# Clemapfel/kmer_index

Hardware: AMD Instinct MI355X
Metric: M queries/sec, DNA4 k=10 exact-match batch search, 1e8-bp text (higher is better)
Workload: dtype u32/u64

## Files before the change

### include/kmx.h

```cpp
#ifndef KMX_H
#define KMX_H

#include <stddef.h>
#include <stdint.h>

#ifdef __cplusplus
extern "C" {
#endif

#define KMX_VERSION 5
#define KMX_MAX_KS 32
#define KMX_MAX_DEVICES 16
#define KMX_QUERY_SIZE_RANGE 10000
#define KMX_SUBK_FANOUT_LIMIT 10000000ull

typedef enum kmx_status {
    KMX_OK = 0,
    KMX_ERR_INVALID_ARGUMENT = 1,
    KMX_ERR_HIP = 2,
    KMX_ERR_OUT_OF_MEMORY = 3,
    KMX_ERR_NO_DEVICE = 4,
    KMX_ERR_TOO_LARGE = 5
} kmx_status;

// ... 34 lines not shown
} kmx_options;

#define KMX_SEARCH_DEFAULT 0u
#define KMX_SEARCH_KEEP_MASKS 1u
#define KMX_SEARCH_COUNT_ONLY 2u
#define KMX_SEARCH_ASYNC 4u
#define KMX_SEARCH_REFERENCE_PLAN 8u

typedef struct kmx_index kmx_index;
typedef struct kmx_result kmx_result;

#define KMX_N_KERNELS 16
typedef struct kmx_kernel_stat {
    const char* name;
    uint64_t launches;
    double total_ms;
} kmx_kernel_stat;

kmx_status kmx_index_build(const uint8_t* ranks, uint64_t n, uint32_t sigma, const uint32_t* ks,
                           uint32_t n_ks, const kmx_options* opts, kmx_index** out);
void kmx_index_free(kmx_index* index);

kmx_status kmx_index_save(const kmx_index* index, const char* path);
kmx_status kmx_index_load(const char* path, const kmx_options* opts, kmx_index** out);

kmx_status kmx_index_info(const kmx_index* index, uint64_t* n, uint32_t* sigma, uint32_t* n_ks,
                          uint32_t* ks , uint32_t* table_kinds ,
                          uint64_t* device_bytes);

kmx_status kmx_index_memory(const kmx_index* index, uint64_t* positions, uint64_t* aligned_copy, uint64_t* cells,
                            uint64_t* prefix_levels, uint64_t* tables);

kmx_status kmx_index_extend_query_size_range(kmx_index* index, uint32_t new_maximum);

kmx_status kmx_plan(const uint32_t* ks, uint32_t n_ks, uint32_t range, uint8_t* use_multi,
                    uint32_t* nk_off, uint32_t* nk_flat, uint64_t cap, uint64_t* n_flat);

kmx_status kmx_plan_engine(const uint32_t* ks, uint32_t n_ks, uint32_t range, uint32_t sigma, uint32_t* k_used);

kmx_status kmx_choose_best_k(const uint64_t* query_lengths, uint64_t n_lengths, uint32_t n_k, uint32_t* ks_out);

uint64_t kmx_fast_pow(uint64_t base, uint8_t exp);

kmx_status kmx_search_batch(const kmx_index* index, const uint8_t* qranks, const uint64_t* qoff,
                            uint64_t nq, uint32_t flags, kmx_result** out);

kmx_status kmx_search_batch_device(const kmx_index* index, const void* d_qranks, const void* d_qoff,
                                   uint64_t nq, uint32_t flags, void* stream, kmx_result** inout);

kmx_status kmx_result_counts(const kmx_result* r, uint64_t* nq, uint64_t* n_hits, uint64_t* n_exact,
                             uint64_t* n_stitch, uint64_t* n_prefix, uint64_t* n_error);
kmx_status kmx_result_view_device(const kmx_result* r, const uint64_t** d_hit_off,
                                  const uint32_t** d_positions, const uint8_t** d_status);
kmx_status kmx_result_view(kmx_result* r, const uint64_t** hit_off, const uint32_t** positions,
                           const uint8_t** status, const uint8_t** kinds);

kmx_status kmx_result_parts(const kmx_result* r, uint32_t* n_parts);
kmx_status kmx_result_part_view_device(const kmx_result* r, uint32_t part, int32_t* device, uint64_t* q_begin, uint64_t* q_end,
                                       const uint64_t** d_hit_off, const uint32_t** d_positions, const uint8_t** d_status);
kmx_status kmx_index_devices(const kmx_index* index, uint32_t* n_devices, int32_t* devices);

kmx_status kmx_result_gather_device(kmx_result* r, int32_t dst_device, const uint64_t** d_hit_off, const uint32_t** d_positions,
                                    const uint8_t** d_status);

kmx_status kmx_result_masks(kmx_result* r, const uint64_t** mask_base, const uint64_t** mask_words,
                            const uint32_t** cand_count, const uint64_t** cand_src);
kmx_status kmx_index_arena_host(const kmx_index* index, const uint32_t** arena, uint64_t* n_elems);

kmx_status kmx_index_bucket_host(const kmx_index* index, uint32_t k, const uint8_t* ranks, const uint32_t** positions,
                                 uint32_t* count);

kmx_status kmx_index_levels(const kmx_index* index, uint32_t* levels);

#define KMX_PATH_INFO 1
typedef struct kmx_index_path_info {
    uint32_t struct_size;
    uint32_t fill_slots;
    uint32_t fill_nontemporal;
    uint32_t rec64;
    uint32_t tiny_cells;
    uint32_t scan_tile;
    uint32_t n_ks;
    uint32_t cell_shift[KMX_MAX_KS];
} kmx_index_path_info;
kmx_status kmx_index_paths(const kmx_index* index, kmx_index_path_info* out);

typedef struct kmx_result_path_info {
    uint32_t struct_size;
    uint32_t small;
    uint32_t lookup_items;
    uint32_t lookup_pairs;
    uint32_t deferred_long;
    uint32_t tile_q_source;
    uint32_t spec_fill;
    uint32_t spec_ok;
    uint32_t fill_blocks;
    uint32_t fill_tiles;
    uint32_t prefix_plain;
    uint32_t prefix_small;
    uint32_t prefix_merge_small;
    uint32_t prefix_mid;
    uint32_t prefix_long;
    uint32_t prefix_large_chunks;
    uint64_t prefix_large_elems;
} kmx_result_path_info;
#define KMX_TILE_Q_NONE 0u
#define KMX_TILE_Q_PARTITION 1u
#define KMX_TILE_Q_SCAN 2u
kmx_status kmx_result_paths(const kmx_result* r, kmx_result_path_info* out);

void kmx_result_free(kmx_result* r);

#define KMX_APPROX_MAX_SUBST 3
#define KMX_APPROX_EDIT 1u
typedef struct kmx_approx_result kmx_approx_result;
kmx_status kmx_search_approx(const kmx_index* index, const uint8_t* qranks, const uint64_t* qoff, uint64_t nq,
                             uint32_t max_subst, uint32_t flags, kmx_approx_result** out);
kmx_status kmx_approx_counts(const kmx_approx_result* r, uint64_t* nq, uint64_t* n_hits, uint64_t* n_candidates,
                             uint32_t* n_chunks);
kmx_status kmx_approx_view(kmx_approx_result* r, const uint64_t** hit_off, const uint32_t** positions,
                           const uint8_t** mismatches, const uint8_t** status);
kmx_status kmx_approx_lengths(kmx_approx_result* r, const uint32_t** lengths);
void kmx_approx_free(kmx_approx_result* r);

#define KMX_APPROX_BOTH_STRANDS 1
kmx_status kmx_search_approx_strands(const kmx_index* index, const uint8_t* qranks, const uint64_t* qoff, uint64_t nq,
                                     uint32_t max_subst, uint32_t flags, const uint8_t* complement,
                                     kmx_approx_result** out);
kmx_status kmx_approx_strands(kmx_approx_result* r, const uint8_t** strands);

#define KMX_APPROX_REPORT 1
#define KMX_APPROX_LOCI 2u
#define KMX_APPROX_BEST 4u
typedef struct kmx_approx_options {
    uint32_t struct_size;
    uint32_t max_subst;
    uint32_t flags;
    uint32_t max_hits;
    const uint8_t* complement;
} kmx_approx_options;
kmx_status kmx_search_approx_opts(const kmx_index* index, const uint8_t* qranks, const uint64_t* qoff, uint64_t nq,
                                  const kmx_approx_options* options, kmx_approx_result** out);
kmx_status kmx_approx_found(kmx_approx_result* r, const uint64_t** found );

kmx_status kmx_index_text(const kmx_index* index, uint8_t* out_ranks, uint64_t n, uint64_t* packed_bytes);

kmx_status kmx_stats_enable(kmx_index* index, int enable);
kmx_status kmx_stats_get(kmx_index* index, kmx_kernel_stat* stats , uint32_t* n);
kmx_status kmx_stats_reset(kmx_index* index);

kmx_status kmx_debug_words(const kmx_index* index, uint64_t* words16);

const char* kmx_last_error(void);
const char* kmx_status_string(kmx_status s);
uint32_t kmx_version(void);

#ifdef __cplusplus
}
#endif
#endif
```

### kmer_index_amd/csrc/kmx_capi.hip

```cpp
#include <hip/hip_runtime.h>

#include <algorithm>
#include <atomic>
#include <cstddef>
#include <cstdio>
#include <cstdlib>
#include <cstring>
#include <memory>
#include <mutex>
#include <string>
#include <system_error>
#include <thread>
#include <vector>

#include "kmx_approx.h"
#include "kmx_host.h"
#include "kmx_kernels.h"

namespace {

thread_local std::string g_err;

kmx_status fail(kmx_status st, const std::string& msg)
{
// ... 74 lines not shown
        }
        p = nullptr; cap = 0; pinned = false;
    }
    template <typename T> T* as() const { return static_cast<T*>(p); }
};

enum KernelId {
    K_LOOKUP = 0, K_SCAN, K_PARTITION, K_FILL, K_VALIDATE, K_COMPACT, K_PREFIX_LEN, K_MERGE_PASS,
    K_PREFIX_SORT_SMALL, K_PREFIX_MERGE_SMALL, K_PREFIX_SORT_BLOCK, K_SMALL, K_PREFIX_BANDS, K_PREFIX_SPLIT, K_COUNT
};
const char* const kKernelNames[K_COUNT] = {
    "k_lookup", "k_scan", "k_partition", "k_fill", "k_validate", "k_compact",
    "k_prefix_len", "k_prefix_merge_pass", "k_prefix_sort_small", "k_prefix_merge_small", "k_prefix_sort_block", "k_small", "k_prefix_bands", "k_prefix_split"};

struct Stats {
    bool enabled = false;
    std::mutex mu;
    struct Pending { int id; hipEvent_t a, b; };
    std::vector<Pending> pending;
    std::vector<hipEvent_t> pool;
    uint64_t launches[K_COUNT] = {};
    double ms[K_COUNT] = {};

    hipEvent_t get()
    {
        if (!pool.empty()) { hipEvent_t e = pool.back(); pool.pop_back(); return e; }
        hipEvent_t e = nullptr;
        (void)hipEventCreate(&e);
        return e;
    }
    void drain()
    {
        for (auto& p : pending) {
            (void)hipEventSynchronize(p.b);
            float t = 0.f;
            if (hipEventElapsedTime(&t, p.a, p.b) == hipSuccess) { ms[p.id] += t; launches[p.id] += 1; }
            pool.push_back(p.a);
            pool.push_back(p.b);
        }
        pending.clear();
    }
    void destroy()
    {
        drain();
        for (auto e : pool) (void)hipEventDestroy(e);
        pool.clear();
    }
};

}

struct ResultPool {
    std::mutex mu;
    std::vector<kmx_result*> idle;
    std::vector<kmx_result*> pending;
    bool closed = false;
};
constexpr size_t kPoolMaxResults = 8;
constexpr size_t kPoolMaxBytes = size_t(256) << 20;
constexpr size_t kSmallView = size_t(256) << 10;

struct kmx_index {
    std::shared_ptr<ResultPool> pool = std::make_shared<ResultPool>();
    int device = 0;
    uint64_t n = 0;
    uint32_t sigma = 0;
    uint32_t range = KMX_QUERY_SIZE_RANGE;
    std::vector<uint32_t> ks;
    std::vector<uint32_t> table_kinds;
    std::vector<void*> allocs;
    uint64_t device_bytes = 0;
    uint64_t bytes_positions = 0, bytes_aligned = 0, bytes_cells = 0, bytes_levels = 0;
    KmxIndexDev* d_index = nullptr;
    KmxIndexDev* d_index_fast = nullptr;
    const KmxPlanEntry* d_plan_fast = nullptr;
    const uint32_t* d_arena = nullptr;
    unsigned long long* d_dbg = nullptr;
    struct ElemSizes { size_t n_offs, n_slots, n_ukeys, n_aoffs; };
    std::vector<ElemSizes> elem_sizes;
    std::vector<uint8_t> tail;
    KmxIndexDev h_header{};
    kmx::FillVariant fill_variant{12, true};
    bool rec32 = true;
    bool tiny_cells = false;
    bool broken = false;
    std::vector<uint32_t> host_arena;
    Stats stats;
    struct HostDir {
        std::once_flag once;
        kmx_status st = KMX_OK;
        std::string err;
        std::vector<uint32_t> offs;
        std::vector<uint64_t> ukeys;
    };
    std::unique_ptr<HostDir[]> host_dirs;
    std::vector<kmx_index*> peers;
    std::unique_ptr<kmx::PackedText> text = std::make_unique<kmx::PackedText>();
    size_t n_replicas() const { return 1 + peers.size(); }
    kmx_index* replica(size_t i) { return i ? peers[i - 1] : this; }
};

struct SearchCtx {
    kmx_index* ix = nullptr;
    const uint8_t* qr = nullptr;
    const uint64_t* qo = nullptr;
    hipStream_t s = nullptr;
    uint64_t tile_cap = 0, spec_tiles = 0;
    bool spec_fill = false;
    bool pending = false;
};

struct kmx_result {
    const kmx_index* index = nullptr;
    int device = 0;
    hipStream_t stream = nullptr;
    uint32_t flags = 0;
    uint64_t nq = 0, n_hits = 0, n_exact = 0, n_stitch = 0, n_prefix = 0, n_error = 0, n_none = 0;
    uint64_t n_mask_words = 0;
    DevBuf src, cnt, c0, aux, key, p1, kind, status, stitch_list, prefix_list, short_list, hit_off, bsum, ctr, tile_q, out,
        mask_words, stitch_hits, plen, poff, ptmp, pitems, pbands, pcuts, pbanded, psplits, ptiles, pscnt, pscratch, pmid, in_qranks, in_qoff;
    unsigned long long* h_ctr = nullptr;
    HostBuf h_hit_off, h_positions, h_status, h_kinds, h_mask_base, h_mask_words, h_cand_count, h_cand_src, h_small;
    uint64_t* v_hit_off = nullptr; uint32_t* v_positions = nullptr; uint8_t* v_status = nullptr; uint8_t* v_kinds = nullptr;
    const uint64_t* m_base = nullptr; const uint64_t* m_words = nullptr; const uint32_t* m_ccnt = nullptr; const uint64_t* m_csrc = nullptr;
    uint32_t ctr_phase = 0;
    bool ctr_clean = false;
    HostBuf mailbox, small_in;
    DevBuf small_xchg;
    bool small_valid = false;
    bool host_valid = false, host_masks_valid = false;
    bool last_had_stitch = false;
    bool last_had_long = false;
    bool last_had_pairs = false;
    struct PathRec { uint32_t small = 0, items = 0, pairs = 0, defer_long = 0, tile_q_source = 0, spec_fill = 0, spec_ok = 0, fill_blocks = 0, fill_tiles = 0;
                     uint32_t p_plain = 0, p_small = 0, p_merge = 0, p_mid = 0, p_long = 0, p_chunks = 0; uint64_t p_elems = 0; };
    PathRec path;
    std::shared_ptr<ResultPool> pool;
    SearchCtx ctx;
    hipEvent_t done = nullptr;
    bool quiesced = true;
    hipStream_t own_stream = nullptr;
    std::vector<kmx_result*> parts;
    std::vector<uint64_t> part_q0;
    std::vector<uint64_t> part_w0;
    bool chunked = false;
    bool host_chunk = false;
    kmx_result* worker = nullptr;
    kmx_result* worker2 = nullptr;
    DevBuf g_hit_off, g_out, g_status;
    int gather_device = -1;
    hipStream_t gather_stream = nullptr;

    size_t device_bytes() const
    {
        size_t b = 0;
        for (const DevBuf* d : {&src, &cnt, &c0, &aux, &key, &p1, &kind, &status, &stitch_list, &prefix_list, &short_list, &hit_off, &bsum, &ctr,
                                &tile_q, &out, &mask_words, &stitch_hits, &plen, &poff, &ptmp, &pitems, &pbands, &pcuts, &pbanded, &psplits, &ptiles, &pscnt, &pscratch, &pmid, &in_qranks, &in_qoff, &small_xchg})
            b += d->cap;
        return b;
    }

    void release()
    {
        for (DevBuf* b : {&src, &cnt, &c0, &aux, &key, &p1, &kind, &status, &stitch_list, &prefix_list, &short_list, &hit_off, &bsum, &ctr,
                          &tile_q, &out, &mask_words, &stitch_hits, &plen, &poff, &ptmp, &pitems, &pbands, &pcuts, &pbanded, &psplits, &ptiles, &pscnt, &pscratch, &pmid, &in_qranks, &in_qoff, &small_xchg})
            b->release();
        for (HostBuf* b : {&h_hit_off, &h_positions, &h_status, &h_kinds, &h_mask_base, &h_mask_words, &h_cand_count, &h_cand_src, &h_small, &mailbox, &small_in})
            b->release();
        if (h_ctr) (void)hipHostFree(h_ctr);
        h_ctr = nullptr;
        if (done) (void)hipEventDestroy(done);
        done = nullptr;
        if (own_stream) (void)hipStreamDestroy(own_stream);
        own_stream = nullptr;
        if (gather_device >= 0) {
            int cur = 0;
            const bool have = hipGetDevice(&cur) == hipSuccess;
            (void)hipSetDevice(gather_device);
            g_hit_off.release(); g_out.release(); g_status.release();
            if (gather_stream) (void)hipStreamDestroy(gather_stream);
            gather_stream = nullptr;
            gather_device = -1;
            if (have) (void)hipSetDevice(cur);
        }
    }
};

namespace {

kmx_result* take_result(kmx_index* ix)
{
    kmx_result* r = nullptr;
    {
        std::lock_guard<std::mutex> lock(ix->pool->mu);
        if (!ix->pool->idle.empty()) { r = ix->pool->idle.back(); ix->pool->idle.pop_back(); }
    }
    if (!r) r = new kmx_result();
    r->pool = ix->pool;
    return r;
}

template <typename F>
void timed(kmx_index* ix, int id, hipStream_t s, F&& launch)
{
    if (!ix->stats.enabled) { launch(); return; }
    std::lock_guard<std::mutex> lock(ix->stats.mu);
    hipEvent_t a = ix->stats.get(), b = ix->stats.get();
    (void)hipEventRecord(a, s);
    launch();
    (void)hipEventRecord(b, s);
    ix->stats.pending.push_back({id, a, b});
}

template <typename T>
kmx_status upload(kmx_index* ix, const T* host, size_t count, const T** dev_out)
{
    void* p = nullptr;
    size_t bytes = std::max<size_t>(count * sizeof(T), 16) + 16;
// ... 95 lines not shown
    std::vector<uint64_t> cell_base(n_ks, 0);
    for (uint32_t i = 0; i < n_ks; ++i) {
        const auto& im = images[i];
        cell_shift[i] = cell_shift_for(im.table_kind, im.n_keys, im.npos, im.region, o);
        if (cell_shift[i] && (up32_elems(arena_elems) + (im.n_keys << cell_shift[i]) + 65536) * 4 >= (uint64_t(1) << 32)) cell_shift[i] = 0;
        if (!cell_shift[i]) continue;
        arena_elems = up32_elems(arena_elems);
        cell_base[i] = arena_elems;
        arena_elems += im.n_keys << cell_shift[i];
    }
    if (prebuilt_arena && prebuilt_arena_elems < arena_elems) {
        fail(KMX_ERR_INVALID_ARGUMENT, "internal: the prebuilt arena is smaller than the index layout");
        return bail(KMX_ERR_INVALID_ARGUMENT);
    }
    {
        void* p = prebuilt_arena;
        if (!p) {
            hipError_t e = hipMalloc(&p, arena_elems * 4 + KMX_ARENA_PAD);
            if (e != hipSuccess) { fail(KMX_ERR_OUT_OF_MEMORY, std::string("arena: ") + hipGetErrorString(e)); return bail(KMX_ERR_OUT_OF_MEMORY); }
        }
        ix->allocs.push_back(p);
        ix->device_bytes += arena_elems * 4;
        {
            hipError_t e = hipMemset(static_cast<unsigned char*>(p) + arena_elems * 4, 0xFF, KMX_ARENA_PAD);
            if (e != hipSuccess) { fail(KMX_ERR_HIP, std::string("arena padding: ") + hipGetErrorString(e)); return bail(KMX_ERR_HIP); }
        }
        h.arena = static_cast<const uint32_t*>(p);
        ix->d_arena = h.arena;
    }
    h.arena_elems = arena_elems;
    ix->rec32 = (arena_elems + 65536) * 4 < (uint64_t(1) << 32);
    if (const char* f64 = getenv("KMX_FORCE_REC64")) { if (atoi(f64)) ix->rec32 = false; }
    if (const char* fvs = getenv("KMX_FILL_VARIANT")) {
        int e = atoi(fvs);
        if (e == 4 || e == 8 || e == 12 || e == 16) ix->fill_variant = kmx::FillVariant{e, strchr(fvs, 'n') != nullptr};
    }
    {
        void* p = nullptr;
        if (hipMalloc(&p, 16 * 8) == hipSuccess) { (void)hipMemset(p, 0, 16 * 8); ix->allocs.push_back(p); h.dbg = static_cast<unsigned long long*>(p); ix->d_dbg = h.dbg; }
    }
    if (o.keep_host_arena) ix->host_arena.assign(arena_elems, 0);
    uint64_t base = 0;
    for (uint32_t i = 0; i < n_ks; ++i) {
        auto& im = images[i];
        KmxElemDev& el = h.elems[i];
        el.k = im.k; el.table_kind = im.table_kind; el.log2cap = im.log2cap;
        el.n_ukeys = uint32_t(im.d_ukeys_prebuilt ? im.n_ukeys_prebuilt : im.ukeys.size());
        if (im.region > im.npos) base = (base + 31) & ~uint64_t(31);
        el.n_keys = im.n_keys; el.arena_base = base; el.npos = im.npos; el.region = im.region; el.atab = nullptr;
        ix->bytes_positions += im.npos * 4; ix->bytes_aligned += (im.region - im.npos) * 4;
        ix->table_kinds.push_back(im.table_kind);
        ix->elem_sizes.push_back({im.offs.size(), im.slots.size(), im.ukeys.size(),
                                  (im.d_atab_prebuilt || (im.table_kind == KMX_TABLE_DENSE && !im.atab.empty())) ? size_t(im.n_keys + 1) : size_t(0)});
        if (im.positions_on_device) {
            if (o.keep_host_arena) {
                hipError_t e = hipMemcpy(ix->host_arena.data() + base, h.arena + base, im.region * 4, hipMemcpyDeviceToHost);
                if (e != hipSuccess) { fail(KMX_ERR_HIP, std::string("arena download: ") + hipGetErrorString(e)); return bail(KMX_ERR_HIP); }
            }
        } else {
            hipError_t e = hipMemcpy(const_cast<uint32_t*>(h.arena) + base, im.positions.data(), im.region * 4, hipMemcpyHostToDevice);
            if (e != hipSuccess) { fail(KMX_ERR_HIP, std::string("arena upload: ") + hipGetErrorString(e)); return bail(KMX_ERR_HIP); }
            if (o.keep_host_arena) std::copy(im.positions.begin(), im.positions.begin() + im.region, ix->host_arena.begin() + base);
        }
        if (im.d_ukeys_prebuilt) {
            const uint64_t nu = im.n_ukeys_prebuilt, cap = uint64_t(1) << im.log2cap;
            el.offs = im.d_offs_prebuilt; el.ukeys = im.d_ukeys_prebuilt; el.slots = im.d_slots_prebuilt;
            ix->device_bytes += (nu + 1) * 4 + nu * 8 + cap * sizeof(KmxSlot);
            ix->elem_sizes.back() = {size_t(nu + 1), size_t(cap), size_t(nu), size_t(0)};
        } else if (im.d_offs_prebuilt) {
            el.offs = im.d_offs_prebuilt;
            ix->device_bytes += (im.n_keys + 1) * 4;
            ix->elem_sizes.back().n_offs = im.n_keys + 1;
        } else if ((st = upload(ix, im.offs.data(), im.offs.size(), &el.offs)) != KMX_OK) return bail(st);
        if (im.d_atab_prebuilt) {
            el.atab = im.d_atab_prebuilt;
            ix->device_bytes += (im.n_keys + 1) * 4;
        } else if (im.table_kind == KMX_TABLE_DENSE && !im.atab.empty()) {
            if ((st = upload(ix, im.atab.data(), im.atab.size(), &el.atab)) != KMX_OK) return bail(st);
        }
        if (im.table_kind == KMX_TABLE_OPEN && !im.d_ukeys_prebuilt) {
            if ((st = upload(ix, im.slots.data(), im.slots.size(), &el.slots)) != KMX_OK) return bail(st);
            if ((st = upload(ix, im.ukeys.data(), im.ukeys.size(), &el.ukeys)) != KMX_OK) return bail(st);
        }
        el.dir = nullptr; el.dir_shift = 0; el.n_dir = 0;
        if (im.table_kind == KMX_TABLE_OPEN && el.n_ukeys >= 1024) {
            uint32_t key_bits = 1;
            while (key_bits < 64 && (im.n_keys - 1) >> key_bits) ++key_bits;
            uint32_t lg = 0;
            while ((uint64_t(1) << lg) < el.n_ukeys) ++lg;
            const uint32_t D = std::min<uint32_t>(std::min<uint32_t>(20, key_bits), lg > 8 ? lg - 4 : 4);
            void* p = nullptr;
            if (hipMalloc(&p, ((size_t(1) << D) + 1) * 4 + 64) == hipSuccess) {
                ix->allocs.push_back(p);
                ix->device_bytes += ((size_t(1) << D) + 1) * 4;
                el.dir = static_cast<const uint32_t*>(p);
                el.dir_shift = key_bits - D;
                el.n_dir = 1u << D;
                kmx::launch_build_dir(nullptr, el.ukeys, el.n_ukeys, el.dir_shift, el.n_dir, static_cast<uint32_t*>(p));
                hipError_t le = hipGetLastError();
                if (le == hipSuccess) le = hipDeviceSynchronize();
                if (le != hipSuccess) { fail(KMX_ERR_HIP, std::string("key directory: ") + hipGetErrorString(le)); return bail(KMX_ERR_HIP); }
            } else {
                (void)hipGetLastError();
            }
        }
        el.cnt8 = nullptr; el.cell_base = 0; el.cell_shift = 0; el.n_levels = 0;
        if (cell_shift[i]) {
            void* p = nullptr;
            hipError_t ce = hipMalloc(&p, im.n_keys + 64);
            if (ce == hipSuccess) {
                ix->allocs.push_back(p);
                ix->device_bytes += im.n_keys;
                (void)hipMemset(p, 0, im.n_keys + 64);
                kmx::launch_build_cells(nullptr, el.offs, h.arena + base, im.n_keys, cell_shift[i], const_cast<uint32_t*>(h.arena) + cell_base[i],
                                        static_cast<uint8_t*>(p));
                ce = hipGetLastError();
                if (ce == hipSuccess) ce = hipDeviceSynchronize();
            }
            if (ce != hipSuccess) { fail(ce == hipErrorOutOfMemory ? KMX_ERR_OUT_OF_MEMORY : KMX_ERR_HIP, std::string("cells: ") + hipGetErrorString(ce)); return bail(KMX_ERR_HIP); }
            el.cnt8 = static_cast<const uint8_t*>(p);
            if (im.npos <= 4 * im.n_keys) ix->tiny_cells = true;
            ix->bytes_cells += ((im.n_keys << cell_shift[i]) * 4) + im.n_keys;
            el.cell_base = cell_base[i];
            el.cell_shift = cell_shift[i];
            if (o.keep_host_arena) {
                ce = hipMemcpy(ix->host_arena.data() + cell_base[i], h.arena + cell_base[i], (im.n_keys << cell_shift[i]) * 4, hipMemcpyDeviceToHost);
                if (ce != hipSuccess) { fail(KMX_ERR_HIP, std::string("cells download: ") + hipGetErrorString(ce)); return bail(KMX_ERR_HIP); }
            }
        }
        base += im.region;
        im = kmx::ElemImage();
    }
    ix->host_dirs.reset(new kmx_index::HostDir[n_ks]);
    ix->tail.assign(tail_kmax, tail_kmax + kmax);
    if ((st = upload(ix, tail_kmax, kmax, &h.tail)) != KMX_OK) return bail(st);
    {
        std::vector<KmxPlanEntry> plan = kmx::make_plan_entries(ix->ks, range);
        if ((st = upload(ix, plan.data(), plan.size(), &h.plan)) != KMX_OK) return bail(st);
    }
    {
        const KmxIndexDev* d = nullptr;
        if ((st = upload(ix, &h, 1, &d)) != KMX_OK) return bail(st);
        ix->d_index = const_cast<KmxIndexDev*>(d);
        ix->h_header = h;
        std::vector<KmxPlanEntry> fast = kmx::make_fast_plan_entries(ix->ks, range, sigma);
        if ((st = upload(ix, fast.data(), fast.size(), &ix->d_plan_fast)) != KMX_OK) return bail(st);
        if ((st = upload(ix, &h, 1, &d)) != KMX_OK) return bail(st);
        ix->d_index_fast = const_cast<KmxIndexDev*>(d);
        const hipError_t pe = publish_headers(ix);
        if (pe != hipSuccess) { fail(KMX_ERR_HIP, std::string("header: ") + hipGetErrorString(pe)); return bail(KMX_ERR_HIP); }
    }
    *out = ix;
    return KMX_OK;
}

static kmx_status replicate_index(const kmx_index* src, int device, kmx_index** out)
{
    auto* ix = new kmx_index();
    ix->device = device;
    ix->n = src->n; ix->sigma = src->sigma; ix->range = src->range;
    ix->ks = src->ks; ix->table_kinds = src->table_kinds; ix->elem_sizes = src->elem_sizes; ix->tail = src->tail;
    ix->fill_variant = src->fill_variant; ix->rec32 = src->rec32; ix->tiny_cells = src->tiny_cells;
    ix->bytes_positions = src->bytes_positions; ix->bytes_aligned = src->bytes_aligned; ix->bytes_cells = src->bytes_cells; ix->bytes_levels = src->bytes_levels;
    auto bail = [&](kmx_status s) { std::string keep = g_err; kmx_index_free(ix); g_err = keep; return s; };
    hipError_t e = hipSetDevice(device);
    if (e != hipSuccess) { fail(KMX_ERR_NO_DEVICE, std::string("replica device: ") + hipGetErrorString(e)); return bail(KMX_ERR_NO_DEVICE); }
    kmx_status st = KMX_OK;
    auto clone = [&](const void* sp, size_t bytes, size_t pad, const void** dp) -> bool {
        *dp = nullptr;
        if (!sp) return true;
        void* p = nullptr;
        hipError_t e2 = hipMalloc(&p, std::max<size_t>(bytes, 16) + pad);
        if (e2 != hipSuccess) { st = fail(KMX_ERR_OUT_OF_MEMORY, std::string("replica: ") + hipGetErrorString(e2)); return false; }
        ix->allocs.push_back(p);
        ix->device_bytes += bytes;
        if (bytes) {
            e2 = hipMemcpyPeer(p, device, sp, src->device, bytes);
            if (e2 != hipSuccess) { st = fail(KMX_ERR_HIP, std::string("replica copy: ") + hipGetErrorString(e2)); return false; }
        }
        *dp = p;
        return true;
    };
    KmxIndexDev h = src->h_header;
    const void* p = nullptr;
    if (!clone(src->h_header.arena, h.arena_elems * 4 + KMX_ARENA_PAD, 0, &p)) return bail(st);
    h.arena = static_cast<const uint32_t*>(p); ix->d_arena = h.arena;
    if (!clone(src->h_header.tail, h.kmax, 16, &p)) return bail(st);
    h.tail = static_cast<const uint8_t*>(p);
    if (!clone(src->h_header.plan, size_t(h.range) * sizeof(KmxPlanEntry), 16, &p)) return bail(st);
    h.plan = static_cast<const KmxPlanEntry*>(p);
    if (!clone(src->d_plan_fast, src->d_plan_fast ? size_t(h.range) * sizeof(KmxPlanEntry) : 0, 16, &p)) return bail(st);
    ix->d_plan_fast = static_cast<const KmxPlanEntry*>(p);
    {
        void* d = nullptr;
        if (hipMalloc(&d, 16 * 8) == hipSuccess) { (void)hipMemset(d, 0, 16 * 8); ix->allocs.push_back(d); h.dbg = static_cast<unsigned long long*>(d); ix->d_dbg = h.dbg; }
        else { (void)hipGetLastError(); h.dbg = nullptr; }
    }
    for (uint32_t i = 0; i < h.n_ks; ++i) {
        const KmxElemDev& se = src->h_header.elems[i];
        KmxElemDev& de = h.elems[i];
        const auto& sz = src->elem_sizes[i];
        if (!clone(se.offs, sz.n_offs * 4, 16, &p)) return bail(st);
        de.offs = static_cast<const uint32_t*>(p);
        if (!clone(se.atab, sz.n_aoffs * 4, 16, &p)) return bail(st);
        de.atab = static_cast<const uint32_t*>(p);
        if (!clone(se.slots, sz.n_slots * sizeof(KmxSlot), 16, &p)) return bail(st);
        de.slots = static_cast<const KmxSlot*>(p);
        if (!clone(se.ukeys, sz.n_ukeys * 8, 16, &p)) return bail(st);
        de.ukeys = static_cast<const uint64_t*>(p);
        if (!clone(se.dir, se.dir ? (size_t(se.n_dir) + 1) * 4 : 0, 64, &p)) return bail(st);
        de.dir = static_cast<const uint32_t*>(p);
        if (!clone(se.cnt8, se.cnt8 ? size_t(se.n_keys) : 0, 64, &p)) return bail(st);
        de.cnt8 = static_cast<const uint8_t*>(p);
    }
    if (!clone(nullptr, 0, 0, &p)) return bail(st);
    {
        void* d = nullptr;
        e = hipMalloc(&d, sizeof(KmxIndexDev) + 16);
        if (e == hipSuccess) { ix->allocs.push_back(d); e = hipMemcpy(d, &h, sizeof h, hipMemcpyHostToDevice); }
        if (e != hipSuccess) { fail(KMX_ERR_HIP, std::string("replica header: ") + hipGetErrorString(e)); return bail(KMX_ERR_HIP); }
        ix->d_index = static_cast<KmxIndexDev*>(d);
        ix->h_header = h;
        if (ix->d_plan_fast) {
            void* d2 = nullptr;
            e = hipMalloc(&d2, sizeof(KmxIndexDev) + 16);
            if (e == hipSuccess) { ix->allocs.push_back(d2); ix->d_index_fast = static_cast<KmxIndexDev*>(d2); e = publish_headers(ix); }
            if (e != hipSuccess) { fail(KMX_ERR_HIP, std::string("replica header: ") + hipGetErrorString(e)); return bail(KMX_ERR_HIP); }
        }
    }
    *out = ix;
    return KMX_OK;
}

static kmx_status search_finish(kmx_result* r);
static kmx_status add_prefix_levels_impl(kmx_index* ix, const kmx_options& o);
static kmx_status add_prefix_levels(kmx_index* ix, const kmx_options& o)
{
    const kmx::FillVariant keep = ix->fill_variant;
    ix->fill_variant.nt = false;
    const kmx_status st = add_prefix_levels_impl(ix, o);
    ix->fill_variant = keep;
    return st;
}
static kmx_status add_prefix_levels_impl(kmx_index* ix, const kmx_options& o)
{
    int want = o.prefix_levels;
    if (want == 0) {
        want = KMX_DEFAULT_PREFIX_LEVELS;
        if (const char* env = getenv("KMX_PREFIX_LEVELS")) want = atoi(env);
    }
    if (want <= 0) return KMX_OK;
    want = std::min(want, int(KMX_MAX_LEVELS));
    HIP_TRY(hipSetDevice(ix->device));
    const std::vector<KmxPlanEntry> plan = kmx::make_plan_entries(ix->ks, ix->range);
    auto up32w = [](uint64_t v) { return (v + 31) & ~uint64_t(31); };
    for (uint32_t e = 0; e < ix->h_header.n_ks; ++e) {
        for (int L = 1; L <= want; ++L) {
            KmxIndexDev& h = ix->h_header;
            KmxElemDev& el = h.elems[e];
            if (el.table_kind != KMX_TABLE_DENSE || uint32_t(L) >= el.k) break;
            const uint32_t m = el.k - uint32_t(L);
            if (m >= ix->range || plan[m].scheme != KMX_SCHEME_SINGLE || plan[m].elem != e) break;
            const uint64_t nq = h.pw[m];
            const uint64_t n_pos = h.n - m + 1;
            if (nq > (uint64_t(1) << 26) || nq * m > (uint64_t(1) << 30)) break;
            const uint64_t offs_at = up32w(h.arena_elems), base = up32w(offs_at + nq + 1), new_elems = base + n_pos;
            if ((new_elems + 65536) * 4 >= (uint64_t(1) << 32)) break;
            size_t free_b = 0, total_b = 0;
            if (hipMemGetInfo(&free_b, &total_b) != hipSuccess) { (void)hipGetLastError(); break; }
            if (double(free_b) < 1.25 * double(new_elems * 4 + n_pos * 4 + nq * (m + 96)) + double(size_t(256) << 20)) break;
            void *d_q = nullptr, *d_off = nullptr, *grown = nullptr;
            kmx_result* r = nullptr;
            auto cleanup = [&] {
                if (d_q) (void)hipFree(d_q);
                if (d_off) (void)hipFree(d_off);
                if (grown) (void)hipFree(grown);
                if (r) kmx_result_free(r);
            };
            auto soft_fail = [&] { (void)hipGetLastError(); cleanup(); };
            if (hipMalloc(&d_q, nq * m + 64) != hipSuccess || hipMalloc(&d_off, (nq + 1) * 8) != hipSuccess) { soft_fail(); break; }
            kmx::launch_all_kmers(nullptr, m, h.sigma, nq, static_cast<uint8_t*>(d_q), static_cast<uint64_t*>(d_off));
            if (hipGetLastError() != hipSuccess || hipDeviceSynchronize() != hipSuccess) { soft_fail(); break; }
            kmx_status st = kmx_search_batch_device(ix, d_q, d_off, nq, KMX_SEARCH_DEFAULT, nullptr, &r);
            if (st == KMX_ERR_OUT_OF_MEMORY) { soft_fail(); break; }
            if (st != KMX_OK) { cleanup(); return st; }
            if (r->n_hits != n_pos || r->n_error) {
                cleanup();
                return fail(KMX_ERR_HIP, "prefix level: the lists of all " + std::to_string(m) + "-mers do not add up to the text's positions");
            }
            if (hipMalloc(&grown, new_elems * 4 + KMX_ARENA_PAD) != hipSuccess) { soft_fail(); break; }
            uint32_t* g = static_cast<uint32_t*>(grown);
            hipError_t he = hipMemcpy(g, h.arena, h.arena_elems * 4, hipMemcpyDeviceToDevice);
            if (he == hipSuccess) he = hipMemset(g + h.arena_elems, 0, (base - h.arena_elems) * 4);
            if (he == hipSuccess) {
                kmx::launch_narrow_offsets(nullptr, r->hit_off.as<uint64_t>(), nq + 1, g + offs_at);
                he = hipGetLastError();
// ... 505 lines not shown
            ix->broken = true;
            restore();
            return fail(KMX_ERR_HIP, first_err + "; the previous planner tables could not be restored on every replica: the index is unusable");
        }
        g_err = first_err;
    }
    restore();
    return st;
}

kmx_status kmx_index_arena_host(const kmx_index* ix, const uint32_t** arena, uint64_t* n_elems)
{
    if (!ix || !arena) return fail(KMX_ERR_INVALID_ARGUMENT, "kmx_index_arena_host: NULL argument");
    if (ix->host_arena.empty()) return fail(KMX_ERR_INVALID_ARGUMENT, "index was built without keep_host_arena");
    *arena = ix->host_arena.data();
    if (n_elems) *n_elems = ix->host_arena.size();
    return KMX_OK;
}

kmx_status kmx_index_bucket_host(const kmx_index* cix, uint32_t k, const uint8_t* ranks, const uint32_t** positions, uint32_t* count)
{
    if (!cix || !ranks || !positions || !count) return fail(KMX_ERR_INVALID_ARGUMENT, "kmx_index_bucket_host: NULL argument");
    *positions = nullptr; *count = 0;
    kmx_index* ix = const_cast<kmx_index*>(cix);
    if (ix->host_arena.empty()) return fail(KMX_ERR_INVALID_ARGUMENT, "kmx_index_bucket_host: index was built without keep_host_arena");
    size_t e = 0;
    while (e < ix->ks.size() && ix->ks[e] != k) ++e;
    if (e == ix->ks.size() || !ix->host_dirs) return fail(KMX_ERR_INVALID_ARGUMENT, "kmx_index_bucket_host: the index holds no element for k = " + std::to_string(k));
    uint64_t h = 0;
    for (uint32_t i = 0; i < k; ++i) {
        if (ranks[i] >= ix->sigma) return fail(KMX_ERR_INVALID_ARGUMENT, "kmx_index_bucket_host: a letter outside the alphabet");
        h = h * ix->sigma + ranks[i];
    }
    const KmxElemDev& el = ix->h_header.elems[e];
    kmx_index::HostDir& hd = ix->host_dirs[e];
    std::call_once(hd.once, [&] {
        int cur = 0;
        const bool have = hipGetDevice(&cur) == hipSuccess;
        hipError_t he = hipSetDevice(ix->device);
        try {
            hd.offs.resize(ix->elem_sizes[e].n_offs);
            if (el.table_kind == KMX_TABLE_OPEN) hd.ukeys.resize(ix->elem_sizes[e].n_ukeys);
        } catch (const std::bad_alloc&) {
            hd.st = KMX_ERR_OUT_OF_MEMORY; hd.err = "kmx_index_bucket_host: host allocation failed";
        }
        if (hd.st == KMX_OK) {
            if (he == hipSuccess && !hd.offs.empty()) he = hipMemcpy(hd.offs.data(), el.offs, hd.offs.size() * 4, hipMemcpyDeviceToHost);
            if (he == hipSuccess && !hd.ukeys.empty()) he = hipMemcpy(hd.ukeys.data(), el.ukeys, hd.ukeys.size() * 8, hipMemcpyDeviceToHost);
            if (he != hipSuccess) { hd.st = KMX_ERR_HIP; hd.err = std::string("kmx_index_bucket_host: table download: ") + hipGetErrorString(he); }
        }
        if (have) (void)hipSetDevice(cur);
    });
    if (hd.st != KMX_OK) return fail(hd.st, hd.err);
    uint64_t g = h;
    if (el.table_kind == KMX_TABLE_OPEN) {
        const auto it = std::lower_bound(hd.ukeys.begin(), hd.ukeys.end(), h);
        if (it == hd.ukeys.end() || *it != h) return KMX_OK;
        g = uint64_t(it - hd.ukeys.begin());
    }
    if (g + 1 >= hd.offs.size()) return KMX_OK;
    const uint32_t a = hd.offs[g], b = hd.offs[g + 1];
    if (b == a) return KMX_OK;
    *positions = ix->host_arena.data() + el.arena_base + a;
    *count = b - a;
    return KMX_OK;
}

kmx_status kmx_index_levels(const kmx_index* ix, uint32_t* levels)
{
    if (!ix || !levels) return fail(KMX_ERR_INVALID_ARGUMENT, "kmx_index_levels: NULL argument");
    for (size_t i = 0; i < ix->ks.size(); ++i) levels[i] = ix->h_header.elems[i].n_levels;
    return KMX_OK;
}

kmx_status kmx_index_paths(const kmx_index* ix, kmx_index_path_info* out)
{
    if (!ix || !out || out->struct_size < sizeof(uint32_t)) return fail(KMX_ERR_INVALID_ARGUMENT, "kmx_index_paths: NULL argument or no struct_size");
    const kmx::FillVariant fv = kmx::effective_fill_variant(ix->fill_variant, ix->rec32);
    kmx_index_path_info v{};
    v.fill_slots = uint32_t(fv.e); v.fill_nontemporal = fv.nt; v.rec64 = !ix->rec32; v.tiny_cells = ix->tiny_cells;
    v.scan_tile = uint32_t(kmx::scan_tile());
    v.n_ks = uint32_t(ix->ks.size());
    for (size_t i = 0; i < ix->ks.size(); ++i) v.cell_shift[i] = ix->h_header.elems[i].cnt8 ? ix->h_header.elems[i].cell_shift : 0u;
    v.struct_size = std::min<uint32_t>(out->struct_size, uint32_t(sizeof v));
    memcpy(out, &v, v.struct_size);
    return KMX_OK;
}

kmx_status kmx_result_paths(const kmx_result* r, kmx_result_path_info* out)
{
    if (!r || !out || out->struct_size < sizeof(uint32_t)) return fail(KMX_ERR_INVALID_ARGUMENT, "kmx_result_paths: NULL argument or no struct_size");
    if (!r->parts.empty()) return fail(KMX_ERR_INVALID_ARGUMENT, "kmx_result_paths: a result of several parts has no single search to report");
    if (r->ctx.pending) { kmx_status fs = search_finish(const_cast<kmx_result*>(r)); if (fs != KMX_OK) return fs; }
    kmx_result_path_info v{};
    v.small = r->path.small; v.lookup_items = r->path.items; v.lookup_pairs = r->path.pairs; v.deferred_long = r->path.defer_long;
    v.tile_q_source = r->path.tile_q_source; v.spec_fill = r->path.spec_fill; v.spec_ok = r->path.spec_ok;
    v.fill_blocks = r->path.fill_blocks; v.fill_tiles = r->path.fill_tiles;
    v.prefix_plain = r->path.p_plain; v.prefix_small = r->path.p_small; v.prefix_merge_small = r->path.p_merge; v.prefix_mid = r->path.p_mid;
    v.prefix_long = r->path.p_long; v.prefix_large_chunks = r->path.p_chunks; v.prefix_large_elems = r->path.p_elems;
    v.struct_size = std::min<uint32_t>(out->struct_size, uint32_t(sizeof v));
    memcpy(out, &v, v.struct_size);
    return KMX_OK;
}

kmx_status kmx_debug_words(const kmx_index* ix, uint64_t* words16)
{
    if (!ix || !words16 || !ix->d_dbg) return fail(KMX_ERR_INVALID_ARGUMENT, "kmx_debug_words: NULL argument");
    HIP_TRY(hipSetDevice(ix->device));
    HIP_TRY(hipDeviceSynchronize());
    HIP_TRY(hipMemcpy(words16, ix->d_dbg, 16 * 8, hipMemcpyDeviceToHost));
    return KMX_OK;
}

kmx_status kmx_stats_enable(kmx_index* ix, int enable)
{
    if (!ix) return fail(KMX_ERR_INVALID_ARGUMENT, "kmx_stats_enable: index is NULL");
    for (kmx_index* peer : ix->peers) (void)kmx_stats_enable(peer, enable);
    std::lock_guard<std::mutex> lock(ix->stats.mu);
    ix->stats.enabled = enable != 0;
    return KMX_OK;
}

kmx_status kmx_stats_get(kmx_index* ix, kmx_kernel_stat* stats, uint32_t* n)
{
    if (!ix || !stats || !n) return fail(KMX_ERR_INVALID_ARGUMENT, "kmx_stats_get: NULL argument");
    {
        std::lock_guard<std::mutex> lock(ix->stats.mu);
        (void)hipSetDevice(ix->device);
        ix->stats.drain();
        for (int i = 0; i < K_COUNT; ++i) stats[i] = kmx_kernel_stat{kKernelNames[i], ix->stats.launches[i], ix->stats.ms[i]};
    }
    for (kmx_index* peer : ix->peers) {
        std::lock_guard<std::mutex> lock(peer->stats.mu);
        (void)hipSetDevice(peer->device);
        peer->stats.drain();
        for (int i = 0; i < K_COUNT; ++i) { stats[i].launches += peer->stats.launches[i]; stats[i].total_ms += peer->stats.ms[i]; }
    }
    if (!ix->peers.empty()) (void)hipSetDevice(ix->device);
    *n = K_COUNT;
    return KMX_OK;
}

kmx_status kmx_stats_reset(kmx_index* ix)
{
    if (!ix) return fail(KMX_ERR_INVALID_ARGUMENT, "kmx_stats_reset: index is NULL");
    for (kmx_index* peer : ix->peers) (void)kmx_stats_reset(peer);
    std::lock_guard<std::mutex> lock(ix->stats.mu);
    (void)hipSetDevice(ix->device);
    ix->stats.drain();
    for (int i = 0; i < K_COUNT; ++i) { ix->stats.launches[i] = 0; ix->stats.ms[i] = 0; }
    return KMX_OK;
}

kmx_status kmx_search_batch_device(const kmx_index* cix, const void* d_qranks, const void* d_qoff, uint64_t nq,
                                   uint32_t flags, void* stream, kmx_result** inout)
{
    if (!cix || !inout) return fail(KMX_ERR_INVALID_ARGUMENT, "kmx_search_batch_device: NULL argument");
    if (nq && (!d_qranks || !d_qoff)) return fail(KMX_ERR_INVALID_ARGUMENT, "kmx_search_batch_device: NULL query buffers");
    if (nq >= 0xFFFFFFFFull) return fail(KMX_ERR_INVALID_ARGUMENT, "kmx_search_batch_device: at most 2^32-2 queries per batch");
    kmx_index* ix = const_cast<kmx_index*>(cix);
    if (ix->broken) return fail(KMX_ERR_HIP, "the index is unusable: a failed kmx_index_extend_query_size_range left its replicas inconsistent");
    if (!ix->peers.empty() && nq) {
        hipPointerAttribute_t attr{};
        if (hipPointerGetAttributes(&attr, d_qranks) != hipSuccess) { (void)hipGetLastError(); return fail(KMX_ERR_INVALID_ARGUMENT, "kmx_search_batch_device: d_qranks is not a device pointer"); }
        kmx_index* pick = nullptr;
        for (size_t i = 0; i < ix->n_replicas() && !pick; ++i)
            if (ix->replica(i)->device == attr.device) pick = ix->replica(i);
        if (!pick) return fail(KMX_ERR_INVALID_ARGUMENT, "kmx_search_batch_device: the queries live on a device that holds no replica of this index");
        ix = pick;
    }
    HIP_TRY(hipSetDevice(ix->device));
    hipStream_t s = static_cast<hipStream_t>(stream);
    const uint8_t* qr = static_cast<const uint8_t*>(d_qranks);
    const uint64_t* qo = static_cast<const uint64_t*>(d_qoff);

    kmx_result* r = *inout;
    if (r && !r->parts.empty()) return fail(KMX_ERR_INVALID_ARGUMENT, "kmx_search_batch_device: the result handle belongs to a multi-device search");
    if (r && r->device != ix->device && r->device_bytes())
        return fail(KMX_ERR_INVALID_ARGUMENT, "kmx_search_batch_device: the result handle holds buffers on another device");
    if (!r) { r = take_result(ix); *inout = r; }
    else if (r->ctx.pending) { kmx_status fs = search_finish(r); if (fs != KMX_OK) return fs; }
    r->index = ix;
    r->device = ix->device;
    r->stream = s;
    (void)hipGetLastError();
    r->flags = flags;
    r->nq = nq;
    r->n_hits = r->n_exact = r->n_stitch = r->n_prefix = r->n_error = r->n_none = r->n_mask_words = 0;
    r->host_valid = r->host_masks_valid = false;
    r->small_valid = false;
    r->path = kmx_result::PathRec{};
    r->quiesced = false;
    if (!r->h_ctr) HIP_TRY(hipHostMalloc(reinterpret_cast<void**>(&r->h_ctr), KMX_CTR_COUNT * sizeof(unsigned long long), hipHostMallocDefault));
    HIP_TRY(r->hit_off.ensure((nq + 1) * 8));
    if (nq == 0) {
        HIP_TRY(hipMemsetAsync(r->hit_off.p, 0, 8, s));
        return KMX_OK;
    }
    HIP_TRY(r->src.ensure(nq * 8));
    HIP_TRY(r->cnt.ensure(nq * 4));
    HIP_TRY(r->c0.ensure(nq * 4));
    HIP_TRY(r->aux.ensure(nq * 8));
    HIP_TRY(r->key.ensure(nq * 8));
    HIP_TRY(r->p1.ensure(nq * 8));
    HIP_TRY(r->kind.ensure(nq));
    HIP_TRY(r->status.ensure(nq));
    HIP_TRY(r->stitch_list.ensure(nq * 4));
    HIP_TRY(r->prefix_list.ensure(nq * 4));
    HIP_TRY(r->short_list.ensure(nq * 4));
    HIP_TRY(r->bsum.ensure(std::max(kmx::scan_blocks(nq), kmx::lookup_blocks(nq, 4)) * 8));
    if (r->ctr.cap < 2 * KMX_CTR_COUNT * sizeof(unsigned long long)) {
        HIP_TRY(r->ctr.ensure(2 * KMX_CTR_COUNT * sizeof(unsigned long long)));
        HIP_TRY(hipMemsetAsync(r->ctr.p, 0, 2 * KMX_CTR_COUNT * sizeof(unsigned long long), s));
        r->ctr_phase = 0;
        r->ctr_clean = true;
    }
    kmx::QueryDesc d{r->src.as<uint64_t>(), r->cnt.as<uint32_t>(), r->c0.as<uint32_t>(), r->aux.as<uint64_t>(),
                     r->key.as<uint64_t>(), r->p1.as<uint64_t>(), r->kind.as<uint8_t>(), r->status.as<uint8_t>(),
                     r->stitch_list.as<uint32_t>(), r->prefix_list.as<uint32_t>(), r->short_list.as<uint32_t>(), nullptr};
    if (!r->ctr_clean) {
        HIP_TRY(hipMemsetAsync(r->ctr.p, 0, 2 * KMX_CTR_COUNT * sizeof(unsigned long long), s));
        r->ctr_clean = true;
    }
    r->ctr_phase ^= 1u;
    auto* ctr = r->ctr.as<unsigned long long>() + r->ctr_phase * KMX_CTR_COUNT;
    auto* ctr_next = r->ctr.as<unsigned long long>() + (r->ctr_phase ^ 1u) * KMX_CTR_COUNT;
    const KmxIndexDev* dix = header_for(ix, flags);

    static const int force_items = getenv("KMX_LOOKUP_ITEMS") ? atoi(getenv("KMX_LOOKUP_ITEMS")) : 0;
    const bool pairs = force_items ? force_items == -4 : r->last_had_pairs;
    const int items = force_items ? (force_items == 8 ? 8 : 4) : (!pairs && ix->tiny_cells) ? 8 : 4;
    const bool defer_long = r->last_had_long;
    const uint32_t lflags = (flags & ~KMX_SEARCH_INTERNAL_DEFER_LONG) | (defer_long ? KMX_SEARCH_INTERNAL_DEFER_LONG : 0u);
    r->path.items = uint32_t(items); r->path.pairs = pairs; r->path.defer_long = defer_long;
    timed(ix, K_LOOKUP, s, [&] {
        kmx::launch_lookup(s, items, pairs, dix, qr, qo, nq, d, ctr, r->bsum.as<uint64_t>(), lflags);
        if (defer_long) kmx::launch_lookup_long(s, dix, qr, qo, nq, d, ctr, flags);
    });
    const kmx::FillVariant fv = kmx::effective_fill_variant(ix->fill_variant, ix->rec32);
    const uint64_t tile = kmx::fill_tile(fv);
    const uint64_t tile_cap = r->tile_q.cap / 4;
    bool published = false;
    timed(ix, K_SCAN, s, [&] {
        published = kmx::launch_scan_tiles(s, d.cnt, nq, r->bsum.as<uint64_t>(), r->hit_off.as<uint64_t>(), ctr + KMX_CTR_TOTAL_HITS, tile,
                                           tile_cap >= 2 ? tile_cap - 1 : 0, tile_cap >= 2 ? r->tile_q.as<uint32_t>() : nullptr, items,
                                           kmx::CounterPub{ctr, ctr_next, r->h_ctr});
    });
    r->ctr_clean = published;
    const uint64_t spec_tiles = std::min<uint64_t>(tile_cap >= 2 ? tile_cap - 1 : 0, (r->out.cap / 4) / tile);
    const bool spec_fill = !(flags & KMX_SEARCH_COUNT_ONLY) && !r->last_had_stitch && spec_tiles > 0 && spec_tiles < 0x7FFFFFFFull;
    if (spec_fill)
        timed(ix, K_FILL, s, [&] {
            kmx::launch_fill(s, fv, ix->rec32, dix, ix->d_arena, r->hit_off.as<uint64_t>(), r->tile_q.as<uint32_t>(),
                             ctr + KMX_CTR_TOTAL_HITS, spec_tiles, d, r->out.as<uint32_t>());
        });
    r->path.spec_fill = spec_fill;
    if (!published) HIP_TRY(hipMemcpyAsync(r->h_ctr, ctr, KMX_CTR_COUNT * sizeof(unsigned long long), hipMemcpyDeviceToHost, s));
    r->ctx = SearchCtx{ix, qr, qo, s, tile_cap, spec_tiles, spec_fill, true};
    if (flags & KMX_SEARCH_ASYNC) {
        if (!r->done) HIP_TRY(hipEventCreateWithFlags(&r->done, hipEventDisableTiming));
        HIP_TRY(hipEventRecord(r->done, s));
        r->pool = ix->pool;
        std::lock_guard<std::mutex> lock(ix->pool->mu);
        ix->pool->pending.push_back(r);
        return KMX_OK;
    }
    return search_finish(r);
}

static kmx_status search_finish(kmx_result* r)
{
    if (!r->ctx.pending) return KMX_OK;
    r->ctx.pending = false;
    kmx_index* ix = r->ctx.ix;
    if (r->flags & KMX_SEARCH_ASYNC) {
        std::lock_guard<std::mutex> lock(ix->pool->mu);
        auto& pend = ix->pool->pending;
        pend.erase(std::remove(pend.begin(), pend.end(), r), pend.end());
    }
    const uint8_t* qr = r->ctx.qr;
    const uint64_t* qo = r->ctx.qo;
    hipStream_t s = r->ctx.s;
    const uint64_t nq = r->nq, tile_cap = r->ctx.tile_cap, spec_tiles = r->ctx.spec_tiles;
    const uint32_t flags = r->flags;
    const bool spec_fill = r->ctx.spec_fill;
    HIP_TRY(hipSetDevice(r->device));
    if (r->done && (flags & KMX_SEARCH_ASYNC)) HIP_TRY(hipEventSynchronize(r->done));
    else HIP_TRY(hipStreamSynchronize(s));
    kmx::QueryDesc d{r->src.as<uint64_t>(), r->cnt.as<uint32_t>(), r->c0.as<uint32_t>(), r->aux.as<uint64_t>(),
                     r->key.as<uint64_t>(), r->p1.as<uint64_t>(), r->kind.as<uint8_t>(), r->status.as<uint8_t>(),
                     r->stitch_list.as<uint32_t>(), r->prefix_list.as<uint32_t>(), r->short_list.as<uint32_t>(), nullptr};
    auto* ctr = r->ctr.as<unsigned long long>() + r->ctr_phase * KMX_CTR_COUNT;
    const KmxIndexDev* dix = header_for(ix, flags);
    const kmx::FillVariant fv = kmx::effective_fill_variant(ix->fill_variant, ix->rec32);
    const uint64_t tile = kmx::fill_tile(fv);
    auto scan_hits = [&] {
        timed(ix, K_SCAN, s, [&] {
            kmx::launch_scan_tiles(s, d.cnt, nq, r->bsum.as<uint64_t>(), r->hit_off.as<uint64_t>(), ctr + KMX_CTR_TOTAL_HITS, tile,
                                   tile_cap >= 2 ? tile_cap - 1 : 0, tile_cap >= 2 ? r->tile_q.as<uint32_t>() : nullptr, 0);
        });
    };
    const uint64_t n_stitch_groups = r->h_ctr[KMX_CTR_STITCH], n_stitch_tiny = r->h_ctr[KMX_CTR_STITCH_TINY];
    const uint64_t n_stitch_short = r->h_ctr[KMX_CTR_STITCH_SHORT];
    const uint64_t n_stitch_pending = n_stitch_groups + n_stitch_tiny + n_stitch_short;
    r->n_stitch = n_stitch_pending + r->h_ctr[KMX_CTR_STITCH_RESOLVED];
    r->last_had_stitch = n_stitch_pending != 0;
    r->last_had_long = r->h_ctr[KMX_CTR_LONG] != 0;
    r->last_had_pairs = r->n_stitch != 0;
    const uint64_t n_prefix_small = r->h_ctr[KMX_CTR_PREFIX], n_prefix_big = r->h_ctr[KMX_CTR_PREFIX_BIG];
    r->n_prefix = n_prefix_small + n_prefix_big + r->h_ctr[KMX_CTR_PREFIX_PLAIN];
    r->n_error = r->h_ctr[KMX_CTR_ERROR];
    r->n_none = r->h_ctr[KMX_CTR_NONE];
    r->n_mask_words = r->h_ctr[KMX_CTR_MASK_WORDS];
    r->n_exact = nq - r->n_stitch - r->n_prefix - r->n_error - r->n_none;
    const uint64_t prefix_elems = r->h_ctr[KMX_CTR_PREFIX_ELEMS];
    const uint64_t max_runs = r->h_ctr[KMX_CTR_MAX_RUNS];
    {
        const uint64_t n_merge = r->h_ctr[KMX_CTR_PREFIX_MERGE], n_mid = r->h_ctr[KMX_CTR_PREFIX_MID];
        r->path.p_plain = uint32_t(r->h_ctr[KMX_CTR_PREFIX_PLAIN]);
        r->path.p_merge = uint32_t(n_merge);
        r->path.p_small = uint32_t(n_prefix_small - std::min(n_prefix_small, n_merge));
        r->path.p_mid = uint32_t(n_mid);
        r->path.p_long = uint32_t(n_prefix_big - std::min(n_prefix_big, n_mid));
        r->path.p_chunks = uint32_t(prefix_elems ? max_runs : 0);
        r->path.p_elems = prefix_elems;
    }

    if (n_stitch_pending) {
        HIP_TRY(r->mask_words.ensure(r->n_mask_words * 8));
        static const bool no_survivors = getenv("KMX_NO_STITCH_HITS") != nullptr;
        const uint64_t n_more = r->h_ctr[KMX_CTR_STITCH_MORE];
        if ((!(flags & KMX_SEARCH_COUNT_ONLY) || n_more) && !no_survivors && r->stitch_hits.ensure(r->n_mask_words * 64 * 4) == hipSuccess)
            d.stitch_hits = r->stitch_hits.as<uint32_t>();
        else
            (void)hipGetLastError();
        timed(ix, K_VALIDATE, s, [&] {
            kmx::launch_validate(s, dix, ix->d_arena, qr, qo, d, n_stitch_groups, n_more, n_stitch_tiny, d.stitch_list + (nq - n_stitch_tiny),
                                 n_stitch_short, r->mask_words.as<uint64_t>(), !(flags & KMX_SEARCH_KEEP_MASKS));
        });
        scan_hits();
        HIP_TRY(hipMemcpyAsync(r->h_ctr, ctr, KMX_CTR_COUNT * sizeof(unsigned long long), hipMemcpyDeviceToHost, s));
        HIP_TRY(hipStreamSynchronize(s));
    }
    r->n_hits = r->h_ctr[KMX_CTR_TOTAL_HITS];
    if (flags & KMX_SEARCH_COUNT_ONLY) return KMX_OK;

    const uint64_t total = r->n_hits;
    if (total == 0) {
        r->path.spec_ok = spec_fill;
        r->path.fill_blocks = uint32_t(spec_fill ? spec_tiles : 0);
        return KMX_OK;
    }
    const uint64_t n_tiles = (total + tile - 1) / tile;
    if (n_tiles >= 0x7FFFFFFFull) return fail(KMX_ERR_INVALID_ARGUMENT, "kmx_search_batch_device: result too large, split the batch");
    HIP_TRY(r->out.ensure(total * 4));
    HIP_TRY(r->tile_q.ensure((n_tiles + 1) * 4));
    uint32_t* out = r->out.as<uint32_t>();
    const uint64_t* hit_off = r->hit_off.as<uint64_t>();
    const bool spec_ok = spec_fill && n_stitch_pending == 0 && n_tiles <= spec_tiles;
    r->path.spec_ok = spec_ok;
    r->path.fill_tiles = uint32_t(n_tiles);
    r->path.fill_blocks = uint32_t(spec_ok ? spec_tiles : n_tiles);
    r->path.tile_q_source = (!spec_ok && n_tiles + 1 > tile_cap) ? KMX_TILE_Q_PARTITION : KMX_TILE_Q_SCAN;
    if (!spec_ok) {
        if (n_tiles + 1 > tile_cap)
            timed(ix, K_PARTITION, s, [&] { kmx::launch_partition(s, hit_off, nq, tile, n_tiles, r->tile_q.as<uint32_t>()); });
        timed(ix, K_FILL, s, [&] {
            kmx::launch_fill(s, fv, ix->rec32, dix, ix->d_arena, hit_off, r->tile_q.as<uint32_t>(), ctr + KMX_CTR_TOTAL_HITS, n_tiles, d, out);
        });
    }
    if (n_stitch_pending && !d.stitch_hits)
        timed(ix, K_COMPACT, s, [&] {
            if (n_stitch_groups) kmx::launch_compact(s, ix->d_arena, d, n_stitch_groups, r->mask_words.as<uint64_t>(), hit_off, out);
            if (n_stitch_tiny) {
                kmx::QueryDesc dt = d;
                dt.stitch_list = d.stitch_list + (nq - n_stitch_tiny);
                kmx::launch_compact(s, ix->d_arena, dt, n_stitch_tiny, r->mask_words.as<uint64_t>(), hit_off, out);
            }
            if (n_stitch_short) {
                kmx::QueryDesc dt = d;
                dt.stitch_list = d.short_list;
                kmx::launch_compact(s, ix->d_arena, dt, n_stitch_short, r->mask_words.as<uint64_t>(), hit_off, out);
            }
        });

    kmx::QueryDesc d_big = d;
    d_big.prefix_list = d.prefix_list + (nq - n_prefix_big);
    const uint64_t n_prefix_merge = r->h_ctr[KMX_CTR_PREFIX_MERGE];
    if (n_prefix_small > n_prefix_merge)
        timed(ix, K_PREFIX_SORT_SMALL, s, [&] { kmx::launch_prefix_sort_small(s, dix, qo, d, n_prefix_small, hit_off, ix->d_arena, out); });
    if (n_prefix_merge)
        timed(ix, K_PREFIX_MERGE_SMALL, s, [&] { kmx::launch_prefix_merge_small(s, dix, qo, d, n_prefix_small, hit_off, ix->d_arena, out); });
    if (n_prefix_big) {
        const bool large = max_runs > 1 && prefix_elems > 0;
        const uint64_t np = n_prefix_big, T = kmx::prefix_merge_tile();
        const uint64_t max_tiles = large ? prefix_elems / T + np : 0;
        const uint64_t n_mid = r->h_ctr[KMX_CTR_PREFIX_MID], n_long = np > n_mid ? np - n_mid : 0;
        static const bool no_bands = getenv("KMX_NO_BANDS") != nullptr;
        static const bool no_split = getenv("KMX_NO_SPLIT") != nullptr || no_bands;
        const bool split_ok = large && !no_split;
        const uint64_t n_large_max = prefix_elems / KMX_PSORT_BLOCK_CAP + 1;
// ... 987 lines not shown
```

### kmer_index_amd/csrc/kmx_kernels.h

```cpp
#pragma once
#include <hip/hip_runtime.h>
#include <stdint.h>
#include "kmx_types.h"


namespace kmx {

struct QueryDesc {
    uint64_t* src;
    uint32_t* cnt;
    uint32_t* c0;
    uint64_t* aux;
    uint64_t* key;
    uint64_t* p1;
    uint8_t* kind;
    uint8_t* status;
    uint32_t* stitch_list;
    uint32_t* prefix_list;
    uint32_t* short_list;
    uint32_t* stitch_hits;
};

uint64_t lookup_blocks(uint64_t nq, int items);
void launch_lookup(hipStream_t s, int items, bool pairs, const KmxIndexDev* ix, const uint8_t* qranks, const uint64_t* qoff,
                   uint64_t nq, const QueryDesc& d, unsigned long long* ctr, uint64_t* block_hits, uint32_t flags);
void launch_lookup_long(hipStream_t s, const KmxIndexDev* ix, const uint8_t* qranks, const uint64_t* qoff, uint64_t nq, const QueryDesc& d,
                        unsigned long long* ctr, uint32_t flags);
void launch_validate(hipStream_t s, const KmxIndexDev* ix, const uint32_t* arena, const uint8_t* qranks, const uint64_t* qoff,
                     const QueryDesc& d, uint64_t n_stitch, uint64_t n_more, uint64_t n_tiny, const uint32_t* tiny_list, uint64_t n_short,
                     uint64_t* mask_words, bool direct);
void launch_small(hipStream_t s, const KmxIndexDev* ix, const uint32_t* arena, unsigned char* mailbox, const KmxSmallLayout& layout, uint32_t n_blocks,
                  const KmxSmallArgs& args, uint32_t nq_total, unsigned long long* xchg, uint32_t flags);
uint64_t scan_blocks(uint64_t n);
void launch_build_dir(hipStream_t s, const uint64_t* d_ukeys, uint64_t n_ukeys, uint32_t shift, uint32_t n_dir, uint32_t* d_dir);
void launch_build_cells(hipStream_t s, const uint32_t* d_offs, const uint32_t* d_region, uint64_t n_keys, uint32_t cell_shift,
                        uint32_t* d_cells, uint8_t* d_cnt8);

struct SparseTables {
    uint64_t* d_ukeys = nullptr;
    uint32_t* d_offs = nullptr;
    KmxSlot* d_slots = nullptr;
    uint64_t n_ukeys = 0;
    uint32_t log2cap = 0;
};
hipError_t sort_kmer_positions(hipStream_t s, const uint8_t* d_text, uint64_t n, uint32_t k, uint32_t sigma, uint32_t key_bits,
                               uint32_t* d_positions);
hipError_t build_sparse_element(hipStream_t s, const uint8_t* d_text, uint64_t n, uint32_t k, uint32_t sigma, uint32_t key_bits,
                                uint32_t* d_positions, SparseTables* out);
hipError_t sort_pairs_u64(hipStream_t s, uint64_t* keys_a, uint32_t* vals_a, uint64_t* keys_b, uint32_t* vals_b, uint64_t n, uint32_t key_bits,
                          bool* in_b);
void launch_scan(hipStream_t s, const uint32_t* in, uint64_t n, uint64_t* bsum, uint64_t* out,
                 unsigned long long* total_out);
struct FillVariant {
    int e;
    bool nt;
};
struct CounterPub {
    const unsigned long long* cur = nullptr;
    unsigned long long* next = nullptr;
    unsigned long long* host = nullptr;
};
bool launch_scan_tiles(hipStream_t s, const uint32_t* in, uint64_t n, uint64_t* bsum, uint64_t* out,
                       unsigned long long* total_out, uint64_t tile, uint64_t n_tiles_cap, uint32_t* tile_q, int lookup_items,
                       const CounterPub& pub = CounterPub());
FillVariant effective_fill_variant(const FillVariant& v, bool rec32);
uint64_t scan_tile();
uint64_t fill_tile(const FillVariant& v);
void launch_partition(hipStream_t s, const uint64_t* off, uint64_t nq, uint64_t tile, uint64_t n_tiles, uint32_t* tile_q);
void launch_fill(hipStream_t s, const FillVariant& v, bool rec32, const KmxIndexDev* ix, const uint32_t* arena, const uint64_t* hit_off,
                 const uint32_t* tile_q, const unsigned long long* total_dev, uint64_t n_tiles, const QueryDesc& d, uint32_t* out);
void launch_compact(hipStream_t s, const uint32_t* arena, const QueryDesc& d, uint64_t n_stitch,
                    const uint64_t* mask_words, const uint64_t* hit_off, uint32_t* out);
void launch_prefix_len(hipStream_t s, const QueryDesc& d, uint64_t n_prefix, const uint32_t* banded, uint32_t* plen);
void launch_build_phase1(hipStream_t s, const uint8_t* d_text, uint64_t n, uint32_t k, uint32_t sigma, uint64_t n_keys,
                         uint32_t* d_hist, uint64_t* d_scratch_u64, uint64_t* d_bsum, uint32_t* d_offs, uint32_t* d_cursor,
                         unsigned int* d_info, unsigned long long* d_total);
void launch_build_phase2(hipStream_t s, const uint8_t* d_text, uint64_t n, uint32_t k, uint32_t sigma, uint64_t n_keys,
                         const uint32_t* d_offs, uint32_t* d_hist, uint64_t* d_scratch_u64, uint64_t* d_bsum, uint32_t* d_cursor,
                         unsigned int* d_info, unsigned long long* d_total, uint32_t* d_region, uint32_t* d_aoffs, uint32_t a0,
                         int sort_mode, uint32_t* d_atab, uint32_t region_end);
void launch_bucket_sort_block(hipStream_t s, const uint32_t* d_offs, uint64_t n_keys, uint32_t* d_positions);
void launch_prefix_sort_small(hipStream_t s, const KmxIndexDev* ix, const uint64_t* qoff, const QueryDesc& d, uint64_t n_prefix,
                              const uint64_t* hit_off, const uint32_t* arena, uint32_t* out);
void launch_prefix_merge_small(hipStream_t s, const KmxIndexDev* ix, const uint64_t* qoff, const QueryDesc& d, uint64_t n_prefix,
                               const uint64_t* hit_off, const uint32_t* arena, uint32_t* out);
struct PrefixSplitRoom {
    void* splits; uint64_t cap_splits;
    void* tiles; uint64_t cap_tiles;
    uint32_t* counters; uint64_t cap_counters;
    uint32_t* scratch; uint64_t cap_scratch;
};
void launch_prefix_bands(hipStream_t s, const KmxIndexDev* ix, const uint64_t* qoff, const QueryDesc& d, uint64_t n_prefix, const uint64_t* hit_off,
                         const uint32_t* arena, uint32_t* banded, void* bands, uint64_t cap_bands, uint32_t* cuts, uint64_t cap_cuts,
                         unsigned long long* used, const PrefixSplitRoom& sr);
void launch_prefix_split(hipStream_t s, const PrefixSplitRoom& sr, const unsigned long long* used, const uint32_t* arena, uint32_t* banded, uint64_t n_text,
                         void* items, uint64_t cap_items, unsigned long long* n_other);
uint64_t prefix_split_bytes(int what);
uint64_t prefix_split_target();
uint64_t prefix_split_tile();
void launch_prefix_sort_block(hipStream_t s, const KmxIndexDev* ix, const uint64_t* qoff, const QueryDesc& d, uint64_t n_prefix, uint64_t n_mid,
                              const uint64_t* hit_off, const uint32_t* arena, uint32_t* out, const uint64_t* tile_off, uint32_t* tmp,
                              void* items, uint64_t cap_items, unsigned long long* n_items, const uint32_t* banded, const void* bands, uint64_t cap_bands,
                              const uint32_t* cuts, const unsigned long long* n_bands, const uint32_t* split, void* mid_items, uint64_t n_text,
                              unsigned long long* dbg);
uint64_t prefix_item_bytes();
uint64_t prefix_band_target();
uint64_t prefix_band_min();
uint64_t prefix_band_runs();
void launch_prefix_merge_pass(hipStream_t s, const QueryDesc& d, uint64_t n_prefix, const uint64_t* tile_off, uint64_t max_tiles,
                              const uint64_t* hit_off, uint32_t* out, uint32_t* tmp, uint32_t pass);
uint64_t prefix_merge_tile();
void launch_all_kmers(hipStream_t s, uint32_t m, uint32_t sigma, uint64_t nq, uint8_t* d_qranks, uint64_t* d_qoff);
void launch_narrow_offsets(hipStream_t s, const uint64_t* d_in, uint64_t n, uint32_t* d_out);
void launch_rebase_offsets(hipStream_t s, uint64_t* d_off, uint64_t n, uint64_t add);

}
```

### kmer_index_amd/csrc/kmx_kernels.hip

```cpp
#include <hip/hip_runtime.h>
#include <stdint.h>

#include <algorithm>
#include <atomic>
#include <type_traits>

#include "kmx_kernels.h"

#define KMX_BLOCK 256
#define KMX_WAVE 64
#define KMX_PSORT_PAIR_CAP 512
#ifndef KMX_PSORT_MULTIWAY_RUNS
#define KMX_PSORT_MULTIWAY_RUNS 4
#endif
#define KMX_PM_WAVE_EMAX (((KMX_PSORT_CAP + (KMX_WAVE - KMX_PSORT_MAX_RUNS / 2) - 1) / (KMX_WAVE - KMX_PSORT_MAX_RUNS / 2)) | 1)
#define KMX_PM_WAVE_PAD (KMX_PSORT_MAX_RUNS + KMX_PM_WAVE_EMAX + 5)
#define KMX_PM_TILE 4096
#define KMX_STAGE_CAP 1024
#define KMX_VGROUP 16
#define KMX_VGROUPS (KMX_WAVE / KMX_VGROUP)
#define KMX_VSLICES (64 / KMX_VGROUP)
#define KMX_VSTAGE (1024 / KMX_VGROUPS)
#define KMX_VCH 8

// ... 323 lines not shown
                            all = ranks_ok && extra.cnt != 0;
                            if (all && track) follow(extra, uint32_t(m - k));
                        }
                        if (all && ranks_ok) {
                            kind = KMX_KIND_STITCH; src = first.src; c0 = first.cnt;
                            key = extra.src;
                            p1 = (uint64_t(extra_delta) << 32) | extra.cnt | (P - 1 + (rest ? 1 : 0) > 1 ? KMX_P1_MORE : 0);
                            if (!(flags & KMX_SEARCH_KEEP_MASKS) && stitch_goes_big(first.cnt, extra.cnt)) p1 |= KMX_P1_BIG;
                            if (track) {
                                const uint32_t lo = alive ? uint32_t(__ffs(int(alive))) - 1u : 0u, len = uint32_t(__popc(alive));
                                if ((alive >> lo) == (1u << len) - 1u) {
                                    resolved = true;
                                    src = first.src + lo;
                                    cnt = len;
                                }
                            }
                        }
                    }
                }
            }
        } else {
            uint64_t mm = m;
            bool all = true;
            Run r{0, 0}, extra{0, 0};
            uint32_t extra_delta = 0;
            const uint32_t nparts = pe.nparts;
            for (uint32_t j = 0; j < nparts && all && ranks_ok; ++j) {
                const KmxPlanEntry e = load_plan_chain(ix, mm);
                const KmxElemDev* el = &elems_s[e.elem];
                const uint32_t k = el->k;
                mm -= k;
                uint64_t h;
                ranks_ok = rank_hash(qr + mm, k, sigma, h, qend);
                if (!ranks_ok) break;
                r = probe(el, h);
                if (j == 0) {
                    extra = r; extra_delta = uint32_t(mm);
                    track = !(flags & KMX_SEARCH_KEEP_MASKS) && nparts > 1 && sparse_buckets(el) && r.cnt != 0 && r.cnt <= KMX_VRESOLVE;
                    if (track) {
                        alive = 0;
#pragma unroll
                        for (uint32_t i = 0; i < KMX_VRESOLVE; ++i) {
                            const uint32_t a = ar[r.src + (i < r.cnt ? i : 0u)];
                            cand[i] = a - uint32_t(mm);
                            alive |= uint32_t(i < r.cnt && a >= uint32_t(mm)) << i;
                        }
                    }
                } else if (track && r.cnt) {
                    follow(r, uint32_t(mm));
                }
                all = r.cnt != 0;
            }
            if (all && ranks_ok) {
                if (nparts == 1) { kind = KMX_KIND_EXACT; src = r.src; cnt = r.cnt; }
                else {
                    kind = KMX_KIND_STITCH; src = r.src; c0 = r.cnt;
                    key = extra.src;
                    p1 = (uint64_t(extra_delta) << 32) | extra.cnt | (nparts > 2 ? KMX_P1_MORE : 0);
                    if (!(flags & KMX_SEARCH_KEEP_MASKS) && stitch_goes_big(r.cnt, extra.cnt)) p1 |= KMX_P1_BIG;
                    if (track) {
                        uint32_t fmask = 0;
                        for (uint32_t t = 0; t < r.cnt; ++t) {
                            const uint32_t b = ar[r.src + t];
#pragma unroll
                            for (uint32_t i = 0; i < KMX_VRESOLVE; ++i) fmask |= uint32_t(((alive >> i) & 1u) && cand[i] == b) << t;
                        }
                        const uint32_t lo = fmask ? uint32_t(__ffs(int(fmask))) - 1u : 0u, len = uint32_t(__popc(fmask));
                        if ((fmask >> lo) == (1u << len) - 1u) {
                            resolved = true;
                            src = r.src + lo;
                            cnt = len;
                        }
                    }
                }
            }
        }
        if (!ranks_ok) { status = KMX_Q_BAD_RANK; kind = KMX_KIND_NONE; cnt = 0; }
    }
    o.src = src; o.aux = aux; o.key = key; o.p1 = p1; o.cnt = cnt; o.c0 = c0; o.kind = kind; o.status = status; o.resolved = resolved;
}

struct BlockCounters {
    unsigned int n_long, base_long;
    unsigned int n_stitch, n_stitch_tiny, n_stitch_short, n_resolved, n_prefix, n_prefix_big, n_prefix_merge, n_prefix_mid, n_prefix_plain, n_error, n_none, n_more;
    unsigned long long words, pelems, hits;
    unsigned int max_runs;
    unsigned int base_stitch, base_stitch_tiny, base_stitch_short, base_prefix, base_prefix_big;
    unsigned long long base_words;
    unsigned int max_fan_exp;
    unsigned int small_keys;
};

template <bool SMALL>
__device__ __forceinline__ bool hash16(const u32x4_a1& w, uint32_t len, uint32_t sigma, uint64_t& h)
{
    uint64_t lo = uint64_t(w[0]) | (uint64_t(w[1]) << 32), hi = uint64_t(w[2]) | (uint64_t(w[3]) << 32);
    {
        const uint32_t sh = (16u - len) * 8u;
        const uint32_t s6 = sh & 63u;
        const uint64_t carry = s6 ? lo >> (64u - s6) : 0;
        const uint64_t hi1 = (hi << s6) | carry, lo1 = lo << s6;
        hi = sh >= 128u ? 0 : sh >= 64u ? lo1 : hi1;
        lo = sh >= 64u ? 0 : lo1;
    }
    const uint32_t wd[4] = {uint32_t(lo), uint32_t(lo >> 32), uint32_t(hi), uint32_t(hi >> 32)};
    uint32_t top = 0;
    if (SMALL) {
        uint32_t acc = 0;
#pragma unroll
        for (uint32_t j = 0; j < 16; ++j) {
            const uint32_t r = (wd[j >> 2] >> (8 * (j & 3))) & 0xFFu;
            top = max(top, r);
            acc = __umul24(acc, sigma) + r;
        }
        h = acc;
    } else {
        uint64_t acc = 0;
#pragma unroll
        for (uint32_t j = 0; j < 16; ++j) {
            const uint32_t r = (wd[j >> 2] >> (8 * (j & 3))) & 0xFFu;
            top = max(top, r);
            acc = acc * sigma + r;
        }
        h = acc;
    }
    return top < sigma;
}
__device__ __forceinline__ const char* probe_first_addr(const KmxElemDev* el, uint64_t h)
{
    if (el->table_kind == KMX_TABLE_DENSE)
        return el->cnt8 ? reinterpret_cast<const char*>(el->cnt8 + (h & ~uint64_t(15)))
                        : reinterpret_cast<const char*>((el->atab ? el->atab : el->offs) + h);
    return reinterpret_cast<const char*>(el->slots + slot_hash_dev(h, el->log2cap));
}
__device__ __forceinline__ Run probe_finish(const KmxElemDev* el, uint64_t h, const u32x4_a1& pr)
{
    Run r{0, 0};
    if (el->table_kind == KMX_TABLE_DENSE) {
        if (el->cnt8) {
            const uint32_t b = uint32_t(h) & 15u;
            const uint32_t wsel = (b >> 2) == 0 ? pr[0] : (b >> 2) == 1 ? pr[1] : (b >> 2) == 2 ? pr[2] : pr[3];
            const uint32_t c = (wsel >> ((b & 3u) * 8u)) & 0xFFu;
            if (c != 255u) { r.src = el->cell_base + (h << el->cell_shift); r.cnt = c; }
            else {
                const KMX_GLOBAL uint32_t* offs = as_global(el->offs);
                const uint32_t a = offs[h], e = offs[h + 1];
                r.src = el->arena_base + a; r.cnt = e - a;
            }
        }
        else if (el->atab) { r.src = el->arena_base + (pr[0] & ~31u); r.cnt = atab_count(pr[0], pr[1]); }
        else { r.src = el->arena_base + pr[0]; r.cnt = pr[1] - pr[0]; }
        return r;
    }
    const KMX_GLOBAL KmxSlot* slots = as_global(el->slots);
    const uint64_t mask = (uint64_t(1) << el->log2cap) - 1;
    uint64_t s = slot_hash_dev(h, el->log2cap);
    uint64_t key = uint64_t(pr[0]) | (uint64_t(pr[1]) << 32);
    uint32_t off = pr[2], c = pr[3];
    while (c != 0 && key != h) {
        s = (s + 1) & mask;
        const u64x2 raw = *(const KMX_GLOBAL u64x2*)(slots + s);
        key = raw.x; off = uint32_t(raw.y); c = uint32_t(raw.y >> 32);
    }
    if (c) { r.src = el->arena_base + off; r.cnt = c; }
    return r;
}

#define KMX_PLAN_LDS 256

#ifndef KMX_LOOKUP_OCC
#define KMX_LOOKUP_OCC 4
#endif
template <int ITEMS, bool PAIRS>
__global__ __launch_bounds__(KMX_BLOCK, PAIRS ? KMX_LOOKUP_OCC : (ITEMS > 4 ? 4 : 5)) void k_lookup(const KmxIndexDev* __restrict__ ix,
                                                      const uint8_t* __restrict__ qranks,
                                                      const uint64_t* __restrict__ qoff, uint64_t nq,
                                                      QueryDesc d, unsigned long long* __restrict__ ctr,
                                                      uint64_t* __restrict__ block_hits, uint32_t flags)
{
    __shared__ BlockCounters bc;
    __shared__ KmxElemDev elems_s[KMX_MAX_KS];
    __shared__ uint32_t plan_s[KMX_PLAN_LDS];
    static_assert(KMX_PLAN_LDS == KMX_BLOCK, "one planner entry per thread");
    if (threadIdx.x == 0) {
        bc.n_long = 0;
        bc.n_stitch = bc.n_stitch_tiny = bc.n_stitch_short = bc.n_resolved = bc.n_prefix = bc.n_prefix_big = bc.n_prefix_merge = bc.n_prefix_mid = bc.n_prefix_plain = bc.n_error = bc.n_none = bc.n_more = 0;
        bc.words = bc.pelems = bc.hits = 0;
        bc.max_runs = 0;
        unsigned int j = 0;
        while (j < 63 && ix->pw[j + 1] <= KMX_SUBK_FANOUT_LIMIT) ++j;
        bc.max_fan_exp = j;
        unsigned int small = ix->sigma < (1u << 24) ? 1u : 0u;
        for (uint32_t e = 0; e < ix->n_ks; ++e) {
            const uint64_t nk = ix->elems[e].n_keys;
            if (nk > (uint64_t(1) << 32) || nk / ix->sigma > (uint64_t(1) << 24)) small = 0;
        }
        bc.small_keys = small;
    }
    {
        const uint32_t n_words = ix->n_ks * uint32_t(sizeof(KmxElemDev) / 8);
        const uint64_t* __restrict__ srcw = reinterpret_cast<const uint64_t*>(ix->elems);
        uint64_t* dstw = reinterpret_cast<uint64_t*>(elems_s);
        for (uint32_t i = threadIdx.x; i < n_words; i += KMX_BLOCK) dstw[i] = srcw[i];
        plan_s[threadIdx.x] = threadIdx.x < ix->range ? ((const KMX_GLOBAL uint32_t*)ix->plan)[threadIdx.x] : 0u;
    }
    const uint8_t* __restrict__ qend = qranks + qoff[nq];
    __syncthreads();

    uint8_t kinds[ITEMS];
    unsigned int locs[ITEMS];
    unsigned long long locw[ITEMS];
    bool done[ITEMS];
    uint64_t my_hits = 0;
    const uint32_t sigma = ix->sigma, range = ix->range;
    const bool small_keys = __builtin_amdgcn_readfirstlane(int(bc.small_keys)) != 0;
    const uint8_t* __restrict__ dummy = reinterpret_cast<const uint8_t*>(ix);

    unsigned int my_resolved = 0, my_err = 0, my_none = 0;
    auto emit = [&](int it, uint64_t q, uint8_t kind, uint8_t status, uint64_t src, uint64_t aux, uint64_t key, uint64_t p1, uint32_t cnt,
                    uint32_t c0, bool resolved) {
        unsigned int loc = 0;
        unsigned long long loc_words = 0;
        if (kind == KMX_KIND_STITCH && !resolved) {
            const uint32_t pc = uint32_t(p1);
            if (min(c0, pc) <= KMX_VTINY && max(c0, pc) <= 2 * KMX_VTINY) {
                loc = atomicAdd(&bc.n_stitch_tiny, 1u) | 0x80000000u;
            } else if (!(p1 & (KMX_P1_MORE | KMX_P1_BIG)) && min(c0, pc) <= KMX_VSHORT && max(c0, pc) <= KMX_VSTAGE) {
                loc = atomicAdd(&bc.n_stitch_short, 1u) | 0x40000000u;
                if (pc < c0) p1 |= KMX_P1_SWAP;
            } else {
                if ((p1 & (KMX_P1_MORE | KMX_P1_BIG)) || stitch_is_wide(p1)) atomicAdd(&bc.n_more, 1u);
                loc = atomicAdd(&bc.n_stitch, 1u);
            }
            loc_words = atomicAdd(&bc.words, (unsigned long long)(uint64_t(c0) / 64 + 1));
        }
        if (kind == KMX_KIND_PREFIX) {
            const uint32_t plen = cnt - uint32_t(__popcll(aux));
            if (c0 < 2 || plen < 2) {
                loc = 0xFFFFFFFFu;
                atomicAdd(&bc.n_prefix_plain, 1u);
            } else if (KMX_PSORT_IS_SMALL(c0, plen)) {
                loc = atomicAdd(&bc.n_prefix, 1u);
                if (KMX_PSORT_IS_MERGE(c0, plen)) atomicAdd(&bc.n_prefix_merge, 1u);
            } else {
                loc = atomicAdd(&bc.n_prefix_big, 1u) | 0x80000000u;
                if (plen <= KMX_PSORT_MID_CAP) atomicAdd(&bc.n_prefix_mid, 1u);
                if (plen > KMX_PSORT_BLOCK_CAP) {
                    atomicAdd(&bc.pelems, (unsigned long long)plen);
                    atomicMax(&bc.max_runs, (plen + KMX_PSORT_BLOCK_CAP - 1) / KMX_PSORT_BLOCK_CAP);
                }
            }
        }
        my_resolved += resolved;
        my_err += status != KMX_Q_OK;
        my_none += status == KMX_Q_OK && kind == KMX_KIND_NONE;
        kinds[it] = !resolved ? kind : uint8_t(KMX_KIND_NONE);
        locs[it] = loc;
        locw[it] = loc_words;
        my_hits += cnt;
        d.src[q] = (kind == KMX_KIND_STITCH && !resolved) ? (src | SRC_SLOW) : (kind == KMX_KIND_PREFIX ? (src | SRC_FLAGS) : src);
        d.cnt[q] = cnt;
        d.kind[q] = kind;
        d.status[q] = status;
        if (kind == KMX_KIND_STITCH) {
            if (!resolved) {
                d.c0[q] = c0;
                d.key[q] = key;
                d.p1[q] = p1;
            }
        } else if (kind == KMX_KIND_PREFIX) {
            d.c0[q] = c0;
            d.aux[q] = aux;
            d.key[q] = key;
        }
    };

    uint64_t qb[ITEMS];
    uint32_t qm[ITEMS];
    uint32_t praw[ITEMS];
#pragma unroll
    for (int it = 0; it < ITEMS; ++it) {
        const uint64_t q = (uint64_t(blockIdx.x) * ITEMS + it) * KMX_BLOCK + threadIdx.x;
        const uint64_t qq = q < nq ? q : nq - 1;
        qb[it] = qoff[qq];
        const uint64_t mlen = qoff[qq + 1] - qb[it];
        qm[it] = mlen > 0xFFFFFFFFull ? 0xFFFFFFFFu : uint32_t(mlen);
        kinds[it] = KMX_KIND_NONE;
        locs[it] = 0;
        locw[it] = 0;
    }
#pragma unroll
    for (int it = 0; it < ITEMS; ++it)
        praw[it] = plan_effective(((const KMX_GLOBAL uint32_t*)ix->plan)[min(qm[it], range - 1)]);

    {
        uint32_t eab[ITEMS];
        bool two[ITEMS];
        u32x4_a1 wa[ITEMS], wb[ITEMS];
        unsigned int n_none = 0, n_err = 0;
#pragma unroll
        for (int it = 0; it < ITEMS; ++it) {
            const uint64_t q = (uint64_t(blockIdx.x) * ITEMS + it) * KMX_BLOCK + threadIdx.x;
            const uint32_t m = qm[it], scheme = praw[it] & 0xFF, e = (praw[it] >> 8) & 0xFF;
            const uint32_t kb = elems_s[e].k;
            const bool live = q < nq && m > 0 && m < range;
            const bool one = live && scheme == KMX_SCHEME_SINGLE && kb == m && m <= 16 && qranks + qb[it] + 16 <= qend;
            bool t = false;
            uint32_t ea = e, off = 0;
            if (PAIRS && live && !one && m < KMX_PLAN_LDS) {
                if (scheme == KMX_SCHEME_SINGLE) {
                    const uint32_t rest = m < 2 * kb ? m - kb : 0u;
                    t = m > kb && m <= 2 * kb && kb <= 16 && (rest == 0 || kb - rest <= bc.max_fan_exp);
                    off = m - kb;
                } else if (scheme == KMX_SCHEME_MULTI && ((praw[it] >> 16) & KMX_PLAN_NPARTS_MASK) == 2 && m > kb) {
                    const uint32_t p2 = plan_s[m - kb];
                    ea = (p2 >> 8) & 0xFF;
                    const uint32_t ka = elems_s[ea].k;
                    t = (p2 & 0xFF) != KMX_SCHEME_NONE && ka + kb == m && ka <= 16 && kb <= 16;
                    off = m - kb;
                }
                t = t && qranks + qb[it] + off + 16 <= qend;
            }
            done[it] = one || t;
            two[it] = t;
            eab[it] = ea | (e << 8) | (off << 16);
            wa[it] = *reinterpret_cast<const u32x4_a1*>(done[it] ? qranks + qb[it] : dummy);
            if (PAIRS) wb[it] = *reinterpret_cast<const u32x4_a1*>(t ? qranks + qb[it] + off : dummy);
        }
        uint64_t ha[ITEMS], hb[ITEMS];
        bool oka[ITEMS], okb[ITEMS];
        u32x4_a1 pa[ITEMS], pb[ITEMS];
#pragma unroll
        for (int it = 0; it < ITEMS; ++it) {
            const KmxElemDev* ela = &elems_s[eab[it] & 0xFF];
            const KmxElemDev* elb = &elems_s[(eab[it] >> 8) & 0xFF];
            okb[it] = true; hb[it] = 0;
            if (small_keys) {
                oka[it] = hash16<true>(wa[it], done[it] ? ela->k : 0u, sigma, ha[it]);
                if (PAIRS) okb[it] = hash16<true>(wb[it], two[it] ? elb->k : 0u, sigma, hb[it]);
            } else {
                oka[it] = hash16<false>(wa[it], done[it] ? ela->k : 0u, sigma, ha[it]);
                if (PAIRS) okb[it] = hash16<false>(wb[it], two[it] ? elb->k : 0u, sigma, hb[it]);
            }
            pa[it] = *(const KMX_GLOBAL u32x4_a1*)((done[it] && oka[it]) ? probe_first_addr(ela, ha[it]) : reinterpret_cast<const char*>(dummy));
            if (PAIRS) pb[it] = *(const KMX_GLOBAL u32x4_a1*)((two[it] && okb[it]) ? probe_first_addr(elb, hb[it]) : reinterpret_cast<const char*>(dummy));
        }
        struct Pend {
            bool two, tiny, first_is_short;
            uint8_t kind, status;
            uint64_t src, key, p1;
            uint32_t c0, off, pc;
            u32x4 s0, s1, l0, l1, l2, l3;
        };
        const KMX_GLOBAL uint32_t* ar = as_global(ix->arena);
        auto stage1 = [&](int it) -> Pend {
            Pend P{};
            P.two = false; P.tiny = false; P.first_is_short = true; P.kind = KMX_KIND_NONE; P.status = KMX_Q_OK; P.src = P.key = P.p1 = 0; P.c0 = P.off = P.pc = 0;
            const uint64_t q = (uint64_t(blockIdx.x) * ITEMS + it) * KMX_BLOCK + threadIdx.x;
            Run ra{0, 0}, rb{0, 0};
            if (done[it]) {
                const KmxElemDev* ela = &elems_s[eab[it] & 0xFF];
                if (oka[it]) ra = probe_finish(ela, ha[it], pa[it]);
                if (!PAIRS || !two[it]) {
                    const uint8_t status = oka[it] ? KMX_Q_OK : KMX_Q_BAD_RANK;
                    n_err += status != KMX_Q_OK;
                    n_none += status == KMX_Q_OK && !ra.cnt;
                    d.src[q] = ra.src;
                    d.cnt[q] = ra.cnt;
                    d.kind[q] = ra.cnt ? KMX_KIND_EXACT : KMX_KIND_NONE;
                    d.status[q] = status;
                    my_hits += ra.cnt;
                } else {
                    const KmxElemDev* elb = &elems_s[(eab[it] >> 8) & 0xFF];
                    const uint32_t off = eab[it] >> 16;
                    const bool multi = (praw[it] & 0xFF) == KMX_SCHEME_MULTI;
                    if (okb[it]) rb = probe_finish(elb, hb[it], pb[it]);
                    const bool bad = multi ? (!okb[it] || (rb.cnt != 0 && !oka[it])) : (!oka[it] || (ra.cnt != 0 && !okb[it]));
                    P.two = true;
                    if (bad) {
                        P.status = KMX_Q_BAD_RANK;
                    } else if (ra.cnt != 0 && rb.cnt != 0) {
                        P.kind = KMX_KIND_STITCH; P.src = ra.src; P.c0 = ra.cnt; P.key = rb.src; P.off = off; P.pc = rb.cnt;
                        P.p1 = (uint64_t(off) << 32) | rb.cnt;
                        if (!(flags & KMX_SEARCH_KEEP_MASKS) && stitch_goes_big(ra.cnt, rb.cnt)) P.p1 |= KMX_P1_BIG;
                        P.tiny = !(flags & KMX_SEARCH_KEEP_MASKS) && min(ra.cnt, rb.cnt) <= KMX_VTINY && max(ra.cnt, rb.cnt) <= 2 * KMX_VTINY;
                        P.first_is_short = ra.cnt <= rb.cnt;
                    }
                }
            }
            static_assert(KMX_VTINY == 8, "two 16-byte loads for the shorter bucket, four for the longer");
            if (!PAIRS) return P;
            const uint64_t sa = !P.tiny ? 0 : P.first_is_short ? ra.src : rb.src, la = !P.tiny ? 0 : P.first_is_short ? rb.src : ra.src;
            P.s0 = *reinterpret_cast<const KMX_GLOBAL u32x4_a4*>(ar + sa); P.s1 = *reinterpret_cast<const KMX_GLOBAL u32x4_a4*>(ar + sa + 4);
            P.l0 = *reinterpret_cast<const KMX_GLOBAL u32x4_a4*>(ar + la); P.l1 = *reinterpret_cast<const KMX_GLOBAL u32x4_a4*>(ar + la + 4);
            P.l2 = *reinterpret_cast<const KMX_GLOBAL u32x4_a4*>(ar + la + 8); P.l3 = *reinterpret_cast<const KMX_GLOBAL u32x4_a4*>(ar + la + 12);
            return P;
        };
        auto stage2 = [&](int it, const Pend& P) {
            if (!PAIRS || !P.two) return;
            const uint64_t q = (uint64_t(blockIdx.x) * ITEMS + it) * KMX_BLOCK + threadIdx.x;
            uint64_t src = P.src;
            uint32_t cnt = 0;
            bool resolved = false;
            if (P.tiny) {
                const uint32_t sv[8] = {P.s0.x, P.s0.y, P.s0.z, P.s0.w, P.s1.x, P.s1.y, P.s1.z, P.s1.w};
                const uint32_t lv[16] = {P.l0.x, P.l0.y, P.l0.z, P.l0.w, P.l1.x, P.l1.y, P.l1.z, P.l1.w, P.l2.x, P.l2.y, P.l2.z, P.l2.w, P.l3.x, P.l3.y, P.l3.z, P.l3.w};
                const uint32_t n_s = P.first_is_short ? P.c0 : P.pc, n_l = P.first_is_short ? P.pc : P.c0;
                const uint32_t shift = P.first_is_short ? P.off : 0u - P.off;
                uint32_t lm[16];
#pragma unroll
                for (uint32_t b = 0; b < 16; ++b) lm[b] = b < n_l ? lv[b] : 0xFFFFFFFFu;
                uint32_t met = 0;
                uint32_t last = 0;
#pragma unroll
                for (uint32_t a = 0; a < 8; ++a) {
                    const bool usable = a < n_s && (P.first_is_short || sv[a] >= P.off);
                    const uint32_t x = usable ? sv[a] + shift : 0xFFFFFFFEu;
                    uint32_t diff = 0xFFFFFFFFu;
#pragma unroll
                    for (uint32_t b = 0; b < 16; b += 2) diff = min(diff, min(x ^ lm[b], x ^ lm[b + 1]));
                    const bool hit = diff == 0;
                    met |= uint32_t(hit) << a;
                    last = hit ? x : last;
                }
                const uint32_t n_met = uint32_t(__popc(met));
                if (P.first_is_short) {
                    const uint32_t lo = met ? uint32_t(__ffs(int(met))) - 1u : 0u;
                    if ((met >> lo) == (1u << n_met) - 1u) {
                        resolved = true; src = P.src + lo; cnt = n_met;
                    }
                } else if (n_met <= 1) {
                    uint32_t rank = 0;
#pragma unroll
                    for (uint32_t b = 0; b < 16; ++b) rank += uint32_t(lm[b] < last);
                    resolved = true; src = P.src + (n_met ? rank : 0u); cnt = n_met;
                }
            }
            emit(it, q, P.kind, P.status, src, 0, P.key, P.p1, cnt, P.c0, resolved);
        };
        static_assert(ITEMS == 4 || ITEMS == 8, "the two-in-flight schedule below");
        {
            Pend p0 = stage1(0);
            Pend p1 = stage1(1);
#pragma unroll
            for (int it = 2; it < ITEMS; it += 2) {
                stage2(it - 2, p0);
                p0 = stage1(it);
                stage2(it - 1, p1);
                p1 = stage1(it + 1);
            }
            stage2(ITEMS - 2, p0);
            stage2(ITEMS - 1, p1);
        }
        if (n_err) atomicAdd(&bc.n_error, n_err);
        if (n_none) atomicAdd(&bc.n_none, n_none);
    }

#pragma unroll 1
    for (int it = 0; it < ITEMS; ++it) {
        if (done[it]) continue;
        const uint64_t q = (uint64_t(blockIdx.x) * ITEMS + it) * KMX_BLOCK + threadIdx.x;
        if (q >= nq) continue;
        const uint64_t b = qoff[q];
        const uint64_t m = qoff[q + 1] - b;
        if (m > 0 && m < range) {
            const KmxPlanEntry pe = plan_unpack(plan_effective(m < KMX_PLAN_LDS ? plan_s[m] : ((const KMX_GLOBAL uint32_t*)ix->plan)[m]));
            if (pe.scheme == KMX_SCHEME_SINGLE) {
                const uint32_t k = elems_s[pe.elem].k;
                if (m > uint64_t(k) * KMX_LONG_PARTS) {
                    const unsigned int slot = atomicAdd(&bc.n_long, 1u);
                    if (flags & KMX_SEARCH_INTERNAL_DEFER_LONG) {
                        kinds[it] = 0xFF;
                        locs[it] = slot;
                        continue;
                    }
                }
            }
        }
        LookupOut lo;
        lookup_query(ix, elems_s, qranks + b, m, qend, flags & ~KMX_SEARCH_INTERNAL_DEFER_LONG, lo);
        emit(it, q, lo.kind, lo.status, lo.src, lo.aux, lo.key, lo.p1, lo.cnt, lo.c0, lo.resolved);
    }

    if (my_resolved) atomicAdd(&bc.n_resolved, my_resolved);
    if (my_err) atomicAdd(&bc.n_error, my_err);
    if (my_none) atomicAdd(&bc.n_none, my_none);
    for (int off = 32; off > 0; off >>= 1) my_hits += __shfl_xor(my_hits, off);
    if (lane_id() == 0 && my_hits) atomicAdd(&bc.hits, (unsigned long long)my_hits);
    __syncthreads();
    if (threadIdx.x == 0) {
        if (block_hits) block_hits[blockIdx.x] = bc.hits;
        if (bc.n_stitch | bc.n_stitch_tiny | bc.n_stitch_short) {
            if (bc.n_stitch) bc.base_stitch = (unsigned int)atomicAdd(&ctr[KMX_CTR_STITCH], (unsigned long long)bc.n_stitch);
            if (bc.n_stitch_tiny) bc.base_stitch_tiny = (unsigned int)atomicAdd(&ctr[KMX_CTR_STITCH_TINY], (unsigned long long)bc.n_stitch_tiny);
            if (bc.n_stitch_short) bc.base_stitch_short = (unsigned int)atomicAdd(&ctr[KMX_CTR_STITCH_SHORT], (unsigned long long)bc.n_stitch_short);
            bc.base_words = atomicAdd(&ctr[KMX_CTR_MASK_WORDS], bc.words);
            if (bc.n_more) atomicAdd(&ctr[KMX_CTR_STITCH_MORE], (unsigned long long)bc.n_more);
        }
        if (bc.n_prefix) bc.base_prefix = (unsigned int)atomicAdd(&ctr[KMX_CTR_PREFIX], (unsigned long long)bc.n_prefix);
        if (bc.n_prefix_merge) atomicAdd(&ctr[KMX_CTR_PREFIX_MERGE], (unsigned long long)bc.n_prefix_merge);
        if (bc.n_prefix_mid) atomicAdd(&ctr[KMX_CTR_PREFIX_MID], (unsigned long long)bc.n_prefix_mid);
        if (bc.n_prefix_plain) atomicAdd(&ctr[KMX_CTR_PREFIX_PLAIN], (unsigned long long)bc.n_prefix_plain);
        if (bc.n_prefix_big) {
            bc.base_prefix_big = (unsigned int)atomicAdd(&ctr[KMX_CTR_PREFIX_BIG], (unsigned long long)bc.n_prefix_big);
            if (bc.pelems) atomicAdd(&ctr[KMX_CTR_PREFIX_ELEMS], bc.pelems);
            if (bc.max_runs) atomicMax(&ctr[KMX_CTR_MAX_RUNS], (unsigned long long)bc.max_runs);
        }
        if (bc.n_long) bc.base_long = (unsigned int)atomicAdd(&ctr[KMX_CTR_LONG], (unsigned long long)bc.n_long);
        if (bc.n_resolved) atomicAdd(&ctr[KMX_CTR_STITCH_RESOLVED], (unsigned long long)bc.n_resolved);
        if (bc.n_error) atomicAdd(&ctr[KMX_CTR_ERROR], (unsigned long long)bc.n_error);
        if (bc.n_none) atomicAdd(&ctr[KMX_CTR_NONE], (unsigned long long)bc.n_none);
    }
    __syncthreads();
#pragma unroll
    for (int it = 0; it < ITEMS; ++it) {
        const uint64_t q = (uint64_t(blockIdx.x) * ITEMS + it) * KMX_BLOCK + threadIdx.x;
        if (kinds[it] == 0xFF) {
            d.short_list[nq - 1 - (bc.base_long + locs[it])] = uint32_t(q);
        } else if (kinds[it] == KMX_KIND_STITCH) {
            d.aux[q] = bc.base_words + locw[it];
            if (locs[it] & 0x80000000u) d.stitch_list[nq - 1 - (bc.base_stitch_tiny + (locs[it] & 0x3FFFFFFFu))] = uint32_t(q);
            else if (locs[it] & 0x40000000u) d.short_list[bc.base_stitch_short + (locs[it] & 0x3FFFFFFFu)] = uint32_t(q);
            else d.stitch_list[bc.base_stitch + locs[it]] = uint32_t(q);
        } else if (kinds[it] == KMX_KIND_PREFIX && locs[it] != 0xFFFFFFFFu) {
            if (locs[it] & 0x80000000u) d.prefix_list[nq - 1 - (bc.base_prefix_big + (locs[it] & 0x7FFFFFFFu))] = uint32_t(q);
            else d.prefix_list[bc.base_prefix + locs[it]] = uint32_t(q);
        }
    }
}

__global__ __launch_bounds__(KMX_BLOCK) void k_lookup_long(const KmxIndexDev* __restrict__ ix, const uint8_t* __restrict__ qranks,
                                                           const uint64_t* __restrict__ qoff, uint64_t nq, QueryDesc d,
                                                           unsigned long long* __restrict__ ctr, uint32_t flags)
{
    const uint32_t lane = lane_id();
    const uint64_t wave = (uint64_t(blockIdx.x) * KMX_BLOCK + threadIdx.x) / KMX_WAVE;
    const uint64_t n_waves = uint64_t(gridDim.x) * (KMX_BLOCK / KMX_WAVE);
    const uint64_t n_long = ctr[KMX_CTR_LONG];
    const uint8_t* __restrict__ qend = qranks + qoff[nq];
    const uint32_t sigma = ix->sigma;
    for (uint64_t i = wave; i < n_long; i += n_waves) {
        const uint32_t q = d.short_list[nq - 1 - i];
        const uint64_t b = qoff[q], m = qoff[q + 1] - b;
        const uint8_t* __restrict__ qr = qranks + b;
        const KmxPlanEntry pe = load_plan(ix, m);
        const KmxElemDev* __restrict__ el = &ix->elems[pe.elem];
        const uint32_t k = el->k;
        const uint32_t P = uint32_t(m / k), rest = uint32_t(m % k);
        const bool fan = rest && ix->pw[k - rest] > KMX_SUBK_FANOUT_LIMIT;
        const uint32_t n_parts = P + ((rest && !fan) ? 1u : 0u);
        uint32_t my_stop = 0xFFFFFFFFu;
        Run first{0, 0}, last{0, 0};
        for (uint32_t j = lane; j < n_parts; j += KMX_WAVE) {
            const uint64_t start = j < P ? uint64_t(j) * k : m - k;
            uint64_t h;
            const bool ok = rank_hash(qr + start, k, sigma, h, qend);
            Run r{0, 0};
            if (ok) r = probe(el, h);
            if ((!ok || r.cnt == 0) && my_stop == 0xFFFFFFFFu) my_stop = 2 * j + (ok ? 1u : 0u);
            if (j == 0) first = r;
            if (j == n_parts - 1) last = r;
        }
        uint32_t stop = my_stop;
        for (int off = 32; off > 0; off >>= 1) stop = min(stop, uint32_t(__shfl_xor(int(stop), off)));
        const int last_lane = int((n_parts - 1) % KMX_WAVE);
        const uint64_t last_src = __shfl(last.src, last_lane);
        const uint32_t last_cnt = uint32_t(__shfl(int(last.cnt), last_lane));
        if (lane != 0) continue;
        uint8_t kind = KMX_KIND_NONE, status = KMX_Q_OK;
        if (stop != 0xFFFFFFFFu) {
            if (!(stop & 1u)) status = KMX_Q_BAD_RANK;
        } else if (fan) {
            status = KMX_Q_SUBK_FANOUT;
        } else {
            kind = KMX_KIND_STITCH;
        }
        d.cnt[q] = 0;
        d.kind[q] = kind;
        d.status[q] = status;
        if (kind != KMX_KIND_STITCH) {
            d.src[q] = 0;
            atomicAdd(&ctr[status != KMX_Q_OK ? KMX_CTR_ERROR : KMX_CTR_NONE], 1ull);
            continue;
        }
        const uint32_t c0 = first.cnt, delta = uint32_t(rest ? m - k : uint64_t(P - 1) * k);
        uint64_t p1 = (uint64_t(delta) << 32) | last_cnt | KMX_P1_MORE;
        if (!(flags & KMX_SEARCH_KEEP_MASKS) && stitch_goes_big(c0, last_cnt)) p1 |= KMX_P1_BIG;
        d.src[q] = first.src | SRC_SLOW;
        d.c0[q] = c0;
        d.key[q] = last_src;
        d.p1[q] = p1;
        d.aux[q] = atomicAdd(&ctr[KMX_CTR_MASK_WORDS], (unsigned long long)(uint64_t(c0) / 64 + 1));
        if (min(c0, last_cnt) <= KMX_VTINY && max(c0, last_cnt) <= 2 * KMX_VTINY) {
            d.stitch_list[nq - 1 - atomicAdd(&ctr[KMX_CTR_STITCH_TINY], 1ull)] = q;
// ... 2196 lines not shown
                                                                 const uint64_t* __restrict__ tile_off,
                                                                 const uint64_t* __restrict__ hit_off,
                                                                 uint32_t* __restrict__ out, uint32_t* __restrict__ tmp,
                                                                 uint32_t pass)
{
    constexpr uint32_t T = KMX_PM_TILE, E = KMX_PM_TILE / KMX_BLOCK;
    __shared__ uint32_t buf[T + 2 + E];
    __shared__ uint32_t cut[2];
    const uint64_t b = blockIdx.x;
    if (b >= tile_off[n_prefix]) return;
    const uint64_t i = upper_bound_wave(tile_off, n_prefix + 1, b, lane_id()) - 1;
    const uint32_t q = d.prefix_list[i];
    const uint32_t len = d.cnt[q] - uint32_t(__popcll(d.aux[q]));
    const uint32_t P = prefix_merge_passes(len);
    if (pass >= P) return;
    const bool dst_is_out = ((P - pass) & 1u) != 0;
    uint32_t* __restrict__ s_out = out + hit_off[q];
    uint32_t* __restrict__ s_tmp = tmp + tile_off[i] * T;
    const uint32_t* __restrict__ src = dst_is_out ? s_tmp : s_out;
    uint32_t* __restrict__ dst = dst_is_out ? s_out : s_tmp;
    const uint32_t tid = threadIdx.x;
    const uint64_t G = uint64_t(KMX_PSORT_BLOCK_CAP) << pass;
    const uint64_t o0 = (b - tile_off[i]) * T;
    const uint64_t a_lo = (o0 / (2 * G)) * (2 * G);
    const uint64_t a_hi = min(a_lo + G, uint64_t(len)), b_hi = min(a_hi + G, uint64_t(len));
    const uint32_t na = uint32_t(a_hi - a_lo), nb = uint32_t(b_hi - a_hi);
    const uint32_t d0 = uint32_t(o0 - a_lo), d1 = min(d0 + T, na + nb);
    const uint32_t n_out = d1 - d0;
    if (nb == 0) {
        for (uint32_t t = tid; t < n_out; t += KMX_BLOCK) dst[o0 + t] = src[o0 + t];
        return;
    }
    const uint32_t* __restrict__ A = src + a_lo;
    const uint32_t* __restrict__ B = src + a_hi;
    if (tid < KMX_WAVE) {
        const uint32_t c0 = merge_path_cut_wave(A, na, B, nb, d0, tid);
        if (tid == 0) cut[0] = c0;
    } else if (tid < 2 * KMX_WAVE) {
        const uint32_t c1 = merge_path_cut_wave(A, na, B, nb, d1, tid - KMX_WAVE);
        if (tid == KMX_WAVE) cut[1] = c1;
    }
    __syncthreads();
    const uint32_t a0 = cut[0], a1 = cut[1], b0 = d0 - a0;
    const uint32_t nA = a1 - a0, nB = n_out - nA;
    for (uint32_t t = tid; t < n_out + 2; t += KMX_BLOCK) {
        uint32_t v = KMX_PM_SENT;
        if (t < nA) v = A[a0 + t];
        else if (t > nA && t < n_out + 1) v = B[b0 + (t - nA - 1)];
        buf[t] = v;
    }
    __syncthreads();
    const KMX_LDS uint32_t* lb = (const KMX_LDS uint32_t*)buf;
    const uint32_t dg = min(tid * E, n_out);
    const uint32_t lo = merge_path_cut(lb, nA, lb + (nA + 1), nB, dg);
    uint32_t x[E];
    merge_chunk<int(E), false>(lb + lo, lb + (nA + 1 + dg - lo), nullptr, nullptr, E, x);
    __syncthreads();
#pragma unroll
    for (uint32_t j = 0; j < E; ++j)
        if (dg + j < n_out) buf[dg + j] = x[j];
    __syncthreads();
    for (uint32_t t = tid; t < n_out; t += KMX_BLOCK) dst[o0 + t] = buf[t];
}

static void allow_big_lds(const void* fn, size_t bytes, int which)
{
    static std::atomic<uint64_t> done[3] = {{0}, {0}, {0}};
    int dev = 0;
    if (hipGetDevice(&dev) != hipSuccess) { (void)hipGetLastError(); return; }
    const uint64_t bit = uint64_t(1) << (dev & 63);
    if (done[which].load(std::memory_order_acquire) & bit) return;
    (void)hipFuncSetAttribute(fn, hipFuncAttributeMaxDynamicSharedMemorySize, int(bytes));
    done[which].fetch_or(bit, std::memory_order_release);
}

static inline unsigned int blocks_for(uint64_t n, uint64_t per_block)
{
    uint64_t b = (n + per_block - 1) / per_block;
    return (unsigned int)(b ? b : 1);
}

uint64_t lookup_blocks(uint64_t nq, int items) { return blocks_for(nq, uint64_t(KMX_BLOCK) * uint64_t(items)); }

void launch_lookup(hipStream_t s, int items, bool pairs, const KmxIndexDev* ix, const uint8_t* qranks, const uint64_t* qoff,
                   uint64_t nq, const QueryDesc& d, unsigned long long* ctr, uint64_t* block_hits, uint32_t flags)
{
    const dim3 grid(blocks_for(nq, uint64_t(KMX_BLOCK) * uint64_t(items))), block(KMX_BLOCK);
    if (pairs) hipLaunchKernelGGL((k_lookup<4, true>), grid, block, 0, s, ix, qranks, qoff, nq, d, ctr, block_hits, flags);
    else if (items == 8) hipLaunchKernelGGL((k_lookup<8, false>), grid, block, 0, s, ix, qranks, qoff, nq, d, ctr, block_hits, flags);
    else hipLaunchKernelGGL((k_lookup<4, false>), grid, block, 0, s, ix, qranks, qoff, nq, d, ctr, block_hits, flags);
}

void launch_validate(hipStream_t s, const KmxIndexDev* ix, const uint32_t* arena, const uint8_t* qranks, const uint64_t* qoff,
                     const QueryDesc& d, uint64_t n_stitch, uint64_t n_more, uint64_t n_tiny, const uint32_t* tiny_list, uint64_t n_short,
                     uint64_t* mask_words, bool direct)
{
    if (n_tiny)
        hipLaunchKernelGGL(k_validate_tiny, dim3(blocks_for(n_tiny, KMX_BLOCK)), dim3(KMX_BLOCK), 0, s, ix, arena, qranks, qoff, d, tiny_list,
                           n_tiny, mask_words, direct && d.stitch_hits != nullptr);
    if (n_short) {
        const uint64_t swaves = (n_short + KMX_VGROUPS - 1) / KMX_VGROUPS;
        const unsigned int sblocks = (unsigned int)std::min<uint64_t>((swaves + 3) / 4, 256 * 32);
        hipLaunchKernelGGL(k_validate_short, dim3(sblocks ? sblocks : 1), dim3(KMX_BLOCK), 0, s, arena, d, n_short, mask_words);
    }
    if (!n_stitch) return;
    uint64_t waves = (n_stitch + KMX_VGROUPS - 1) / KMX_VGROUPS;
    unsigned int blocks = (unsigned int)std::min<uint64_t>((waves + 3) / 4, 256 * 32);
    const dim3 grid(blocks ? blocks : 1), block(KMX_BLOCK);
    if (n_more && !d.stitch_hits) {
        hipLaunchKernelGGL(k_validate<true>, grid, block, 0, s, ix, arena, qranks, qoff, d, n_stitch, mask_words);
        return;
    }
    hipLaunchKernelGGL(k_validate<false>, grid, block, 0, s, ix, arena, qranks, qoff, d, n_stitch, mask_words);
    if (n_more) {
        const uint64_t sw = (n_stitch + KMX_VWIDE_SCAN - 1) / KMX_VWIDE_SCAN;
        const unsigned int sblocks = (unsigned int)std::min<uint64_t>((sw + 3) / 4, 256 * 16);
        hipLaunchKernelGGL(k_validate_wide, dim3(sblocks ? sblocks : 1), dim3(KMX_VWIDE_BLOCK), 0, s, arena, d, n_stitch, mask_words);
        hipLaunchKernelGGL(k_validate_more_thread, dim3(blocks_for(n_stitch, KMX_BLOCK)), block, 0, s, ix, arena, qranks, qoff, d, n_stitch,
                           uint32_t(n_more >= KMX_VMORE_THREAD_MANY ? KMX_VMORE_THREAD_PARTS_MANY : KMX_VMORE_THREAD_PARTS), mask_words);
        hipLaunchKernelGGL(k_validate_more, grid, block, 0, s, ix, arena, qranks, qoff, d, n_stitch, mask_words);
        const uint64_t wwaves = (n_stitch + KMX_VWAVE_SCAN - 1) / KMX_VWAVE_SCAN;
        const unsigned int wblocks = (unsigned int)std::min<uint64_t>((wwaves + 3) / 4, 256 * 16);
        hipLaunchKernelGGL(k_validate_wave, dim3(wblocks ? wblocks : 1), block, 0, s, ix, arena, qranks, qoff, d, n_stitch, mask_words);
    }
}

uint64_t scan_blocks(uint64_t n) { return blocks_for(n, KMX_SCAN_TILE); }
uint64_t scan_tile() { return KMX_SCAN_TILE; }

#define KMX_SCAN_FUSED_SPINE_BLOCKS 8192

void launch_scan(hipStream_t s, const uint32_t* in, uint64_t n, uint64_t* bsum, uint64_t* out,
                 unsigned long long* total_out)
{
    const unsigned int nb = blocks_for(n, KMX_SCAN_TILE);
    hipLaunchKernelGGL(k_scan_reduce, dim3(nb), dim3(KMX_BLOCK), 0, s, in, n, bsum);
    if (nb <= KMX_SCAN_FUSED_SPINE_BLOCKS) {
        hipLaunchKernelGGL((k_scan_down<false, 1>), dim3(nb), dim3(KMX_BLOCK), 0, s, in, n, bsum, out, uint64_t(1), uint64_t(0),
                           (uint32_t*)nullptr, total_out, uint64_t(0), CounterPub(), 0u);
        return;
    }
    hipLaunchKernelGGL(k_scan_spine, dim3(1), dim3(KMX_BLOCK), 0, s, bsum, uint64_t(nb), total_out);
    hipLaunchKernelGGL((k_scan_down<false, 0>), dim3(nb), dim3(KMX_BLOCK), 0, s, in, n, bsum, out, uint64_t(1), uint64_t(0),
                       (uint32_t*)nullptr, total_out, uint64_t(0), CounterPub(), 0u);
}

bool launch_scan_tiles(hipStream_t s, const uint32_t* in, uint64_t n, uint64_t* bsum, uint64_t* out,
                       unsigned long long* total_out, uint64_t tile, uint64_t n_tiles_cap, uint32_t* tile_q, int lookup_items,
                       const CounterPub& pub)
{
    const unsigned int nb = blocks_for(n, KMX_SCAN_TILE);
    const bool lookup_sums = lookup_items != 0;
    if (lookup_sums && nb <= KMX_SCAN_FUSED_SPINE_BLOCKS) {
        const uint64_t n_fine = lookup_blocks(n, lookup_items);
        const uint32_t fine = uint32_t(KMX_SCAN_TILE / (KMX_BLOCK * lookup_items));
        if (tile_q)
            hipLaunchKernelGGL((k_scan_down<true, 2>), dim3(nb), dim3(KMX_BLOCK), 0, s, in, n, bsum, out, tile, n_tiles_cap, tile_q, total_out, n_fine, pub, fine);
        else
            hipLaunchKernelGGL((k_scan_down<false, 2>), dim3(nb), dim3(KMX_BLOCK), 0, s, in, n, bsum, out, uint64_t(1), uint64_t(0),
                               (uint32_t*)nullptr, total_out, n_fine, pub, fine);
        return pub.host != nullptr;
    }
    if (!tile_q) { launch_scan(s, in, n, bsum, out, total_out); return false; }
    hipLaunchKernelGGL(k_scan_reduce, dim3(nb), dim3(KMX_BLOCK), 0, s, in, n, bsum);
    if (nb <= KMX_SCAN_FUSED_SPINE_BLOCKS) {
        hipLaunchKernelGGL((k_scan_down<true, 1>), dim3(nb), dim3(KMX_BLOCK), 0, s, in, n, bsum, out, tile, n_tiles_cap, tile_q, total_out, uint64_t(0), CounterPub(), 0u);
        return false;
    }
    hipLaunchKernelGGL(k_scan_spine, dim3(1), dim3(KMX_BLOCK), 0, s, bsum, uint64_t(nb), total_out);
    hipLaunchKernelGGL((k_scan_down<true, 0>), dim3(nb), dim3(KMX_BLOCK), 0, s, in, n, bsum, out, tile, n_tiles_cap, tile_q, total_out, uint64_t(0), CounterPub(), 0u);
    return false;
}

// ... 1115 lines not shown
                                                             uint32_t sigma, uint32_t* __restrict__ cursor,
                                                             uint32_t* __restrict__ positions)
{
    const uint64_t stride = uint64_t(gridDim.x) * KMX_BLOCK;
    for (uint64_t i = uint64_t(blockIdx.x) * KMX_BLOCK + threadIdx.x; i < npos; i += stride)
        positions[atomicAdd(&cursor[kmer_hash_at(text, i, k, sigma)], 1u)] = uint32_t(i);
}

__global__ __launch_bounds__(KMX_BLOCK) void k_bucket_sort_wave(const uint32_t* __restrict__ offs, uint64_t n_keys,
                                                                uint32_t* __restrict__ positions)
{
    __shared__ uint32_t buf[KMX_BLOCK / KMX_WAVE][KMX_PSORT_CAP];
    const uint32_t lane = lane_id(), wv = threadIdx.x / KMX_WAVE;
    const uint64_t wave = (uint64_t(blockIdx.x) * KMX_BLOCK + threadIdx.x) / KMX_WAVE;
    const uint64_t n_waves = uint64_t(gridDim.x) * (KMX_BLOCK / KMX_WAVE);
    auto wsync = [] {
        __builtin_amdgcn_fence(__ATOMIC_RELEASE, "wavefront");
        __builtin_amdgcn_wave_barrier();
        __builtin_amdgcn_fence(__ATOMIC_ACQUIRE, "wavefront");
    };
    for (uint64_t h = wave; h < n_keys; h += n_waves) {
        const uint32_t lo = offs[h], len = offs[h + 1] - lo;
        if (len < 2 || len > KMX_PSORT_CAP) continue;
        uint32_t n2 = 2;
        while (n2 < len) n2 <<= 1;
        uint32_t* __restrict__ seg = positions + lo;
        for (uint32_t t = lane; t < n2; t += KMX_WAVE) buf[wv][t] = t < len ? seg[t] : 0xFFFFFFFFu;
        wsync();
        bitonic_lds(buf[wv], n2, lane, KMX_WAVE, wsync);
        for (uint32_t t = lane; t < len; t += KMX_WAVE) seg[t] = buf[wv][t];
        wsync();
    }
}

__global__ __launch_bounds__(1024) void k_bucket_sort_block(const uint32_t* __restrict__ offs, uint64_t n_keys,
                                                            uint32_t* __restrict__ positions)
{
    extern __shared__ __attribute__((aligned(16))) uint32_t sbuf[];
    const uint32_t tid = threadIdx.x;
    for (uint64_t h = blockIdx.x; h < n_keys; h += gridDim.x) {
        const uint32_t lo = offs[h], len = offs[h + 1] - lo;
        if (len <= KMX_PSORT_CAP || len > KMX_PSORT_BLOCK_CAP) continue;
        uint32_t n2 = 2;
        while (n2 < len) n2 <<= 1;
        uint32_t* __restrict__ seg = positions + lo;
        for (uint32_t t = tid; t < n2; t += 1024) sbuf[t] = t < len ? seg[t] : 0xFFFFFFFFu;
        __syncthreads();
        bitonic_lds(sbuf, n2, tid, 1024u, [] { __syncthreads(); });
        for (uint32_t t = tid; t < len; t += 1024) seg[t] = sbuf[t];
        __syncthreads();
    }
}

void launch_bucket_sort_block(hipStream_t s, const uint32_t* d_offs, uint64_t n_keys, uint32_t* d_positions);

__global__ __launch_bounds__(KMX_BLOCK) void k_build_padded(const uint32_t* __restrict__ offs, uint64_t n_keys,
                                                            uint32_t* __restrict__ padded, unsigned int* __restrict__ present)
{
    const uint64_t h = uint64_t(blockIdx.x) * KMX_BLOCK + threadIdx.x;
    uint32_t c = 0;
    if (h < n_keys) {
        c = offs[h + 1] - offs[h];
        padded[h] = (c + 31u) & ~31u;
    }
    const uint64_t nz = __ballot(c != 0);
    if (lane_id() == 0 && nz) atomicAdd(present, (unsigned int)__popcll(nz));
}

__global__ __launch_bounds__(KMX_BLOCK) void k_build_aoffs(const uint64_t* __restrict__ pscan, uint64_t n_keys, uint32_t a0,
                                                           uint32_t* __restrict__ aoffs)
{
    const uint64_t h = uint64_t(blockIdx.x) * KMX_BLOCK + threadIdx.x;
    if (h < n_keys) aoffs[h] = a0 + uint32_t(pscan[h]);
}

__global__ __launch_bounds__(KMX_BLOCK) void k_build_atab(const uint32_t* __restrict__ offs, const uint32_t* __restrict__ aoffs,
                                                          uint64_t n_keys, uint32_t end, uint32_t* __restrict__ atab)
{
    const uint64_t h = uint64_t(blockIdx.x) * KMX_BLOCK + threadIdx.x;
    if (h < n_keys) atab[h] = (aoffs[h] & ~31u) | ((offs[h + 1] - offs[h]) & 31u);
    else if (h == n_keys) atab[h] = end & ~31u;
}

__global__ __launch_bounds__(KMX_BLOCK) void k_build_aligned_copy(const uint32_t* __restrict__ offs,
                                                                  const uint32_t* __restrict__ aoffs, uint64_t n_keys,
                                                                  uint32_t* __restrict__ region)
{
    const uint32_t lane = lane_id();
    const uint64_t wave = (uint64_t(blockIdx.x) * KMX_BLOCK + threadIdx.x) / KMX_WAVE;
    const uint64_t n_waves = uint64_t(gridDim.x) * (KMX_BLOCK / KMX_WAVE);
    for (uint64_t h = wave; h < n_keys; h += n_waves) {
        const uint32_t lo = offs[h], len = offs[h + 1] - lo, dst = aoffs[h];
        for (uint32_t t = lane; t < len; t += KMX_WAVE) region[dst + t] = region[lo + t];
    }
}

void launch_build_phase1(hipStream_t s, const uint8_t* d_text, uint64_t n, uint32_t k, uint32_t sigma, uint64_t n_keys,
                         uint32_t* d_hist, uint64_t* d_scratch_u64, uint64_t* d_bsum, uint32_t* d_offs, uint32_t* d_cursor,
                         unsigned int* d_info, unsigned long long* d_total)
{
    const uint64_t npos = n - k + 1;
    const unsigned int grid = (unsigned int)std::min<uint64_t>(blocks_for(npos, KMX_BLOCK), 256 * 64);
    (void)hipMemsetAsync(d_hist, 0, n_keys * sizeof(uint32_t), s);
    (void)hipMemsetAsync(d_info, 0, 4 * sizeof(unsigned int), s);
    hipLaunchKernelGGL(k_build_hist, dim3(grid), dim3(KMX_BLOCK), 0, s, d_text, npos, k, sigma, d_hist);
    launch_scan(s, d_hist, n_keys, d_bsum, d_scratch_u64, d_total);
    hipLaunchKernelGGL(k_build_offsets, dim3(blocks_for(n_keys + 1, KMX_BLOCK)), dim3(KMX_BLOCK), 0, s, d_scratch_u64, n_keys, d_offs,
                       d_cursor, d_info);
    hipLaunchKernelGGL(k_build_padded, dim3(blocks_for(n_keys, KMX_BLOCK)), dim3(KMX_BLOCK), 0, s, d_offs, n_keys, d_hist, d_info + 1);
    launch_scan(s, d_hist, n_keys, d_bsum, d_scratch_u64, d_total + 1);
}

void launch_build_phase2(hipStream_t s, const uint8_t* d_text, uint64_t n, uint32_t k, uint32_t sigma, uint64_t n_keys,
                         const uint32_t* d_offs, uint32_t* d_hist, uint64_t* d_scratch_u64, uint64_t* d_bsum, uint32_t* d_cursor,
                         unsigned int* d_info, unsigned long long* d_total, uint32_t* d_region, uint32_t* d_aoffs, uint32_t a0,
                         int sort_mode, uint32_t* d_atab, uint32_t region_end)
{
    const uint64_t npos = n - k + 1;
    const unsigned int grid = (unsigned int)std::min<uint64_t>(blocks_for(npos, KMX_BLOCK), 256 * 64);
    const unsigned int wblocks = (unsigned int)std::min<uint64_t>((n_keys + 3) / 4, 256 * 32);
    if (sort_mode != 2) {
        (void)hipMemcpyAsync(d_cursor, d_offs, n_keys * sizeof(uint32_t), hipMemcpyDeviceToDevice, s);
        hipLaunchKernelGGL(k_build_scatter, dim3(grid), dim3(KMX_BLOCK), 0, s, d_text, npos, k, sigma, d_cursor, d_region);
        hipLaunchKernelGGL(k_bucket_sort_wave, dim3(wblocks ? wblocks : 1), dim3(KMX_BLOCK), 0, s, d_offs, n_keys, d_region);
        if (sort_mode == 1) launch_bucket_sort_block(s, d_offs, n_keys, d_region);
    }
    if (d_aoffs) {
        hipLaunchKernelGGL(k_build_padded, dim3(blocks_for(n_keys, KMX_BLOCK)), dim3(KMX_BLOCK), 0, s, d_offs, n_keys, d_hist, d_info + 1);
        launch_scan(s, d_hist, n_keys, d_bsum, d_scratch_u64, d_total + 1);
        hipLaunchKernelGGL(k_build_aoffs, dim3(blocks_for(n_keys, KMX_BLOCK)), dim3(KMX_BLOCK), 0, s, d_scratch_u64, n_keys, a0, d_aoffs);
        hipLaunchKernelGGL(k_build_aligned_copy, dim3(wblocks ? wblocks : 1), dim3(KMX_BLOCK), 0, s, d_offs, d_aoffs, n_keys, d_region);
        if (d_atab)
            hipLaunchKernelGGL(k_build_atab, dim3(blocks_for(n_keys + 1, KMX_BLOCK)), dim3(KMX_BLOCK), 0, s, d_offs, d_aoffs, n_keys, region_end, d_atab);
    }
}

__global__ __launch_bounds__(KMX_BLOCK) void k_build_dir(const uint64_t* __restrict__ ukeys, uint64_t n_ukeys, uint32_t shift,
                                                         uint32_t n_dir, uint32_t* __restrict__ dir)
{
    const uint64_t j = uint64_t(blockIdx.x) * KMX_BLOCK + threadIdx.x;
    if (j > n_dir) return;
    dir[j] = j == n_dir ? uint32_t(n_ukeys) : uint32_t(lower_bound_dev<uint64_t>(ukeys, n_ukeys, j << shift));
}

__global__ __launch_bounds__(KMX_BLOCK) void k_build_cells(const uint32_t* __restrict__ offs, const uint32_t* __restrict__ region,
                                                           uint64_t n_keys, uint32_t cell_shift, uint32_t* __restrict__ cells,
                                                           uint8_t* __restrict__ cnt8)
{
    const uint64_t i = uint64_t(blockIdx.x) * KMX_BLOCK + threadIdx.x;
    const uint64_t h = i >> cell_shift;
    if (h >= n_keys) return;
    const uint32_t j = uint32_t(i) & ((1u << cell_shift) - 1u);
    const uint32_t lo = offs[h], c = offs[h + 1] - lo;
    const bool fits = c <= (1u << cell_shift);
    cells[i] = (fits && j < c) ? region[lo + j] : 0u;
    if (j == 0) cnt8[h] = fits ? uint8_t(c) : uint8_t(255);
}

void launch_build_cells(hipStream_t s, const uint32_t* d_offs, const uint32_t* d_region, uint64_t n_keys, uint32_t cell_shift,
                        uint32_t* d_cells, uint8_t* d_cnt8)
{
    hipLaunchKernelGGL(k_build_cells, dim3(blocks_for(n_keys << cell_shift, KMX_BLOCK)), dim3(KMX_BLOCK), 0, s, d_offs, d_region, n_keys,
                       cell_shift, d_cells, d_cnt8);
}

void launch_build_dir(hipStream_t s, const uint64_t* d_ukeys, uint64_t n_ukeys, uint32_t shift, uint32_t n_dir, uint32_t* d_dir)
// ... 75 lines not shown
```

### kmer_index_amd/csrc/kmx_types.h

```cpp
#pragma once
#include <stdint.h>
#include "../../include/kmx.h"

#define KMX_MAX_LEVELS 3
#define KMX_DEFAULT_PREFIX_LEVELS 2

struct KmxSlot {
    uint64_t key;
    uint32_t off;
    uint32_t cnt;
};

struct KmxElemDev {
    uint32_t k;
    uint32_t table_kind;
    uint32_t log2cap;
    uint32_t n_ukeys;
    uint64_t n_keys;
    uint64_t arena_base;
    uint64_t npos;
    const uint32_t* offs;
    const KmxSlot* slots;
    const uint64_t* ukeys;
    const uint32_t* atab;
    uint64_t region;
    const uint32_t* dir;
    uint32_t dir_shift;
    uint32_t n_dir;
    const uint8_t* cnt8;
    uint64_t cell_base;
    uint32_t cell_shift;
    uint32_t n_levels;
    uint64_t lvl_offs_at[KMX_MAX_LEVELS];
    uint64_t lvl_base[KMX_MAX_LEVELS];
};

enum { KMX_SCHEME_NONE = 0, KMX_SCHEME_SINGLE = 1, KMX_SCHEME_MULTI = 2, KMX_SCHEME_REPLANNED = 3 };
#define KMX_PLAN_ALT_SHIFT 11
#define KMX_PLAN_NPARTS_MASK ((1u << KMX_PLAN_ALT_SHIFT) - 1u)
struct KmxPlanEntry {
    uint8_t scheme;
    uint8_t elem;
    uint16_t nparts;
};

struct KmxIndexDev {
    uint64_t n;
    uint32_t sigma;
    uint32_t n_ks;
    uint32_t kmax;
    uint32_t range;
    const uint32_t* arena;
    const uint8_t* tail;
    const KmxPlanEntry* plan;
    uint64_t arena_elems;
    unsigned long long* dbg;
    uint64_t pw[64];
    KmxElemDev elems[KMX_MAX_KS];
};

#define KMX_PSORT_IS_SMALL(runs, len) ((len) <= KMX_PSORT_CAP)
#ifndef KMX_PMERGE_MIN_AVG
#define KMX_PMERGE_MIN_AVG 8
#endif
#define KMX_PSORT_IS_MERGE(runs, len)                                                                                   \
    ((len) <= KMX_PSORT_CAP && (runs) >= 2 && (runs) <= KMX_PSORT_MAX_RUNS && !((runs) <= KMX_PMERGE_REG_RUNS && (len) <= KMX_PMERGE_REG_LEN) && \
     (len) >= KMX_PMERGE_MIN_AVG * (runs))
#ifndef KMX_PMERGE_REG_RUNS
#define KMX_PMERGE_REG_RUNS 4
#endif
#ifndef KMX_PMERGE_REG_LEN
#define KMX_PMERGE_REG_LEN 512
#endif
#define KMX_VRESOLVE 4
#define KMX_ARENA_PAD (4096 * 4 + 1024)
#define KMX_VTINY 8
#define KMX_VSHORT 16
#define KMX_PSORT_MAX_RUNS 32
#define KMX_PSORT_CAP 2048
#define KMX_PSORT_BLOCK_CAP 32768
#define KMX_PSORT_MID_CAP 8192

#define KMX_SMALL_NQ 256
#define KMX_SMALL_BLOCKS 32
struct KmxSmallArgs {
    uint16_t nq[KMX_SMALL_BLOCKS];
    uint16_t n_letters[KMX_SMALL_BLOCKS];
};
#define KMX_SMALL_IN_BYTES 8192
#define KMX_SMALL_WCAP 1024
#define KMX_SMALL_WSLOW 32
#define KMX_SMALL_SORT 4096
#define KMX_SMALL_BSLOW 8
#define KMX_SMALL_WORDS (KMX_SMALL_WSLOW * (KMX_SMALL_WCAP / 64 + 1) + KMX_SMALL_BSLOW * (KMX_SMALL_SORT / 64 + 1))
#define KMX_SMALL_POS 49152
struct KmxSmallHeader {
    uint32_t fallback;
    uint32_t nq;
    uint64_t n_hits, n_mask_words;
    uint32_t n_stitch, n_prefix, n_error, n_none;
    uint32_t pad[6];
};
struct KmxSmallLayout {
    uint32_t blocks, off_header, off_hitoff, off_csrc, off_mbase, off_ccnt, off_status, off_kinds, off_words, off_pos, bytes, pad;
};
static inline KmxSmallLayout kmx_small_layout(uint32_t blocks)
{
    KmxSmallLayout L;
    const uint32_t nq = blocks * KMX_SMALL_NQ;
    L.blocks = blocks;
    L.off_header = blocks * KMX_SMALL_IN_BYTES;
    L.off_hitoff = L.off_header + blocks * 64;
    L.off_csrc = L.off_hitoff + (nq + 2) * 8;
    L.off_mbase = L.off_csrc + nq * 8;
    L.off_ccnt = L.off_mbase + nq * 8;
    L.off_status = L.off_ccnt + nq * 4;
    L.off_kinds = L.off_status + nq;
    L.off_words = L.off_kinds + nq;
    L.off_pos = L.off_words + blocks * KMX_SMALL_WORDS * 8;
    L.bytes = L.off_pos + blocks * KMX_SMALL_POS * 4;
    L.pad = 0;
    return L;
}

enum {
    KMX_CTR_STITCH = 1,
    KMX_CTR_PREFIX = 2,
    KMX_CTR_ERROR = 3,
    KMX_CTR_MASK_WORDS = 4,
    KMX_CTR_PREFIX_ELEMS = 5,
    KMX_CTR_MAX_RUNS = 6,
    KMX_CTR_TOTAL_HITS = 7,
    KMX_CTR_NONE = 8,
    KMX_CTR_PREFIX_TOTAL = 9,
    KMX_CTR_STITCH_MORE = 10,
    KMX_CTR_PREFIX_BIG = 11,
    KMX_CTR_STITCH_TINY = 12,
    KMX_CTR_STITCH_RESOLVED = 13,
    KMX_CTR_PREFIX_MERGE = 14,
    KMX_CTR_PREFIX_MID = 15,
    KMX_CTR_PREFIX_PLAIN = 0,
    KMX_CTR_STITCH_SHORT = 16,
    KMX_CTR_LONG = 17,
    KMX_CTR_PSB_MERGE = 18,
    KMX_CTR_PSB_OTHER = 19,
    KMX_CTR_PSB_BANDS = 20,
    KMX_CTR_PSB_CUTS = 21,
    KMX_CTR_PSB_SPLITS = 22,
    KMX_CTR_COUNT = 28
};
#define KMX_LONG_PARTS 256
#define KMX_SEARCH_INTERNAL_DEFER_LONG 0x80000000u
```

### kmer_index_amd/engine.py

```python
import ctypes as C
import os

import numpy as np

from . import build as _build

KMX_MAX_KS = 32
KMX_MAX_DEVICES = 16
KMX_N_KERNELS = 16
TABLE_AUTO, TABLE_OPEN, TABLE_DENSE = 0, 1, 2
SEARCH_DEFAULT, SEARCH_KEEP_MASKS, SEARCH_COUNT_ONLY, SEARCH_ASYNC, SEARCH_REFERENCE_PLAN = 0, 1, 2, 4, 8
KIND_NONE, KIND_EXACT, KIND_STITCH, KIND_PREFIX = 0, 1, 2, 3
Q_OK, Q_TOO_LONG, Q_SUBK_FANOUT, Q_EMPTY_QUERY, Q_BAD_RANK, Q_TOO_SHORT = 0, 1, 2, 3, 4, 5
APPROX_MAX_SUBST = 3
APPROX_EDIT = 1
APPROX_LOCI, APPROX_BEST = 2, 4
TILE_Q_NONE, TILE_Q_PARTITION, TILE_Q_SCAN = 0, 1, 2

EXPORTS = [
    "kmx_index_build", "kmx_index_free", "kmx_index_save", "kmx_index_load", "kmx_index_info", "kmx_index_memory", "kmx_index_arena_host", "kmx_index_extend_query_size_range", "kmx_choose_best_k", "kmx_plan", "kmx_plan_engine", "kmx_fast_pow",
    "kmx_search_batch", "kmx_search_batch_device", "kmx_result_counts", "kmx_result_view_device",
    "kmx_result_view", "kmx_result_masks", "kmx_result_free", "kmx_stats_enable", "kmx_stats_get",
    "kmx_stats_reset", "kmx_debug_words", "kmx_last_error", "kmx_status_string", "kmx_version",
    "kmx_index_devices", "kmx_result_parts", "kmx_result_part_view_device",
    "kmx_index_bucket_host", "kmx_index_levels", "kmx_result_gather_device",
    "kmx_search_approx", "kmx_approx_counts", "kmx_approx_view", "kmx_approx_free", "kmx_index_text",
    "kmx_approx_lengths", "kmx_search_approx_strands", "kmx_approx_strands",
    "kmx_search_approx_opts", "kmx_approx_found",
    "kmx_index_paths", "kmx_result_paths",
]


class KmxError(RuntimeError):
    def __init__(self, status, msg):
        super().__init__(f"kmx status {status}: {msg}")
        self.status = status


class Options(C.Structure):
    _fields_ = [("struct_size", C.c_uint32), ("device", C.c_int32), ("table_kind", C.c_uint32),
                ("n_threads", C.c_uint32), ("query_size_range", C.c_uint32), ("keep_host_arena", C.c_uint32),
                ("host_flatten", C.c_uint32), ("no_aligned_copy", C.c_uint32),
                ("n_devices", C.c_uint32), ("devices", C.c_int32 * KMX_MAX_DEVICES), ("prefix_levels", C.c_int32)]


class ApproxOptions(C.Structure):
    _fields_ = [("struct_size", C.c_uint32), ("max_subst", C.c_uint32), ("flags", C.c_uint32), ("max_hits", C.c_uint32),
                ("complement", C.c_void_p)]


class KernelStat(C.Structure):
    _fields_ = [("name", C.c_char_p), ("launches", C.c_uint64), ("total_ms", C.c_double)]


class IndexPathInfo(C.Structure):
    _fields_ = [("struct_size", C.c_uint32), ("fill_slots", C.c_uint32), ("fill_nontemporal", C.c_uint32), ("rec64", C.c_uint32),
                ("tiny_cells", C.c_uint32), ("scan_tile", C.c_uint32), ("n_ks", C.c_uint32), ("cell_shift", C.c_uint32 * KMX_MAX_KS)]


class ResultPathInfo(C.Structure):
    _fields_ = [("struct_size", C.c_uint32), ("small", C.c_uint32), ("lookup_items", C.c_uint32), ("lookup_pairs", C.c_uint32),
                ("deferred_long", C.c_uint32), ("tile_q_source", C.c_uint32), ("spec_fill", C.c_uint32), ("spec_ok", C.c_uint32),
                ("fill_blocks", C.c_uint32), ("fill_tiles", C.c_uint32),
                ("prefix_plain", C.c_uint32), ("prefix_small", C.c_uint32), ("prefix_merge_small", C.c_uint32), ("prefix_mid", C.c_uint32),
                ("prefix_long", C.c_uint32), ("prefix_large_chunks", C.c_uint32), ("prefix_large_elems", C.c_uint64)]


_lib = None


def lib():
    global _lib
    if _lib is None:
        try:
            import torch
        except ImportError:
            pass
        path = _build.build()
        if not os.path.exists(path):
            raise RuntimeError("libkmx.so is missing and could not be built; the engine has no fallback")
        L = C.CDLL(path)
        vp, u64, u32 = C.c_void_p, C.c_uint64, C.c_uint32
        P = C.POINTER
        L.kmx_index_build.restype = C.c_int
        L.kmx_index_build.argtypes = [vp, u64, u32, vp, u32, P(Options), P(vp)]
        L.kmx_index_free.argtypes = [vp]
        L.kmx_index_save.restype = C.c_int
        L.kmx_index_save.argtypes = [vp, C.c_char_p]
        L.kmx_index_load.restype = C.c_int
        L.kmx_index_load.argtypes = [C.c_char_p, P(Options), P(vp)]
        L.kmx_index_info.restype = C.c_int
        L.kmx_index_info.argtypes = [vp, P(u64), P(u32), P(u32), vp, vp, P(u64)]
        L.kmx_index_memory.restype = C.c_int
        L.kmx_index_memory.argtypes = [vp, P(u64), P(u64), P(u64), P(u64), P(u64)]
        L.kmx_index_arena_host.restype = C.c_int
        L.kmx_index_arena_host.argtypes = [vp, P(vp), P(u64)]
        L.kmx_index_extend_query_size_range.restype = C.c_int
        L.kmx_index_extend_query_size_range.argtypes = [vp, u32]
        L.kmx_choose_best_k.restype = C.c_int
        L.kmx_choose_best_k.argtypes = [vp, u64, u32, vp]
        L.kmx_plan.restype = C.c_int
        L.kmx_plan_engine.restype = C.c_int
        L.kmx_plan_engine.argtypes = [vp, u32, u32, u32, vp]
        L.kmx_plan.argtypes = [vp, u32, u32, vp, vp, vp, u64, P(u64)]
        L.kmx_fast_pow.restype = u64
        L.kmx_fast_pow.argtypes = [u64, C.c_uint8]
        L.kmx_search_batch.restype = C.c_int
        L.kmx_search_batch.argtypes = [vp, vp, vp, u64, u32, P(vp)]
        L.kmx_search_batch_device.restype = C.c_int
        L.kmx_search_batch_device.argtypes = [vp, vp, vp, u64, u32, vp, P(vp)]
        L.kmx_result_counts.restype = C.c_int
        L.kmx_result_counts.argtypes = [vp] + [P(u64)] * 6
        L.kmx_result_view_device.restype = C.c_int
        L.kmx_result_view_device.argtypes = [vp, P(vp), P(vp), P(vp)]
        L.kmx_result_view.restype = C.c_int
        L.kmx_result_view.argtypes = [vp, P(vp), P(vp), P(vp), P(vp)]
        L.kmx_result_masks.restype = C.c_int
        L.kmx_result_masks.argtypes = [vp, P(vp), P(vp), P(vp), P(vp)]
        L.kmx_result_free.argtypes = [vp]
        L.kmx_index_devices.restype = C.c_int
        L.kmx_index_devices.argtypes = [vp, P(u32), vp]
        L.kmx_result_parts.restype = C.c_int
        L.kmx_result_parts.argtypes = [vp, P(u32)]
        L.kmx_result_part_view_device.restype = C.c_int
        L.kmx_result_part_view_device.argtypes = [vp, u32, P(C.c_int32), P(u64), P(u64), P(vp), P(vp), P(vp)]
        L.kmx_index_bucket_host.restype = C.c_int
        L.kmx_index_bucket_host.argtypes = [vp, u32, vp, P(vp), P(u32)]
        L.kmx_index_levels.restype = C.c_int
        L.kmx_index_levels.argtypes = [vp, vp]
        L.kmx_result_gather_device.restype = C.c_int
        L.kmx_result_gather_device.argtypes = [vp, C.c_int32, P(vp), P(vp), P(vp)]
        L.kmx_search_approx.restype = C.c_int
        L.kmx_search_approx.argtypes = [vp, vp, vp, u64, u32, u32, P(vp)]
        L.kmx_approx_counts.restype = C.c_int
        L.kmx_approx_counts.argtypes = [vp, P(u64), P(u64), P(u64), P(u32)]
        L.kmx_approx_view.restype = C.c_int
        L.kmx_approx_view.argtypes = [vp, P(vp), P(vp), P(vp), P(vp)]
        L.kmx_approx_lengths.restype = C.c_int
        L.kmx_approx_lengths.argtypes = [vp, P(vp)]
        L.kmx_approx_free.argtypes = [vp]
        L.kmx_search_approx_strands.restype = C.c_int
        L.kmx_search_approx_strands.argtypes = [vp, vp, vp, u64, u32, u32, vp, P(vp)]
        L.kmx_approx_strands.restype = C.c_int
        L.kmx_approx_strands.argtypes = [vp, P(vp)]
        L.kmx_search_approx_opts.restype = C.c_int
        L.kmx_search_approx_opts.argtypes = [vp, vp, vp, u64, P(ApproxOptions), P(vp)]
        L.kmx_approx_found.restype = C.c_int
        L.kmx_approx_found.argtypes = [vp, P(vp)]
# ... 34 lines not shown

def _check(st):
    if st != 0:
        raise KmxError(st, lib().kmx_last_error().decode())


_COMPLEMENT_CHARS = {4: ("ACGT", "TGCA"), 5: ("ACGNT", "TGCNA"), 15: ("ABCDGHKMNRSTVWY", "TVGHCDMKNYSABWR")}


def complement_table(sigma):
    if sigma not in _COMPLEMENT_CHARS:
        raise ValueError(f"complement_table: no natural complement for an alphabet of {sigma} letters; pass a table")
    chars, comp = _COMPLEMENT_CHARS[sigma]
    return np.array([chars.index(c) for c in comp], np.uint8)


def fast_pow(base, exp):
    return int(lib().kmx_fast_pow(base, exp))


def choose_best_k(lengths, n_k=4):
    lengths = np.ascontiguousarray(lengths, np.uint64)
    out = np.zeros(n_k, np.uint32)
    _check(lib().kmx_choose_best_k(lengths.ctypes.data, lengths.size, n_k, out.ctypes.data))
    return out.tolist()


def plan(ks, rng=10000):
    ks = np.ascontiguousarray(ks, np.uint32)
    multi = np.zeros(rng, np.uint8)
    off = np.zeros(rng + 1, np.uint32)
    n = C.c_uint64()
    _check(lib().kmx_plan(ks.ctypes.data, ks.size, rng, multi.ctypes.data, off.ctypes.data, None, 0, C.byref(n)))
    flat = np.zeros(max(n.value, 1), np.uint32)
    _check(lib().kmx_plan(ks.ctypes.data, ks.size, rng, multi.ctypes.data, off.ctypes.data, flat.ctypes.data, n.value, C.byref(n)))
    return multi.astype(bool), [flat[off[q]:off[q + 1]].tolist() for q in range(rng)]


def plan_engine(ks, sigma, rng=10000):
    ks = np.ascontiguousarray(ks, np.uint32)
    out = np.zeros(rng, np.uint32)
    _check(lib().kmx_plan_engine(ks.ctypes.data, ks.size, rng, int(sigma), out.ctypes.data))
    return out


def _view(ptr, n, dtype):
    if not ptr or n == 0:
        return np.zeros(0, dtype)
    ct = np.ctypeslib.as_ctypes_type(dtype)
    return np.ctypeslib.as_array(C.cast(ptr, C.POINTER(ct)), shape=(int(n),))


class Result:

    def __init__(self):
        self._h = C.c_void_p()
        self._index = None

    def n_parts(self):
        n = C.c_uint32()
        _check(lib().kmx_result_parts(self._h, C.byref(n)))
        return int(n.value)

    def part_device_ptrs(self, part):
        dev, qb, qe = C.c_int32(), C.c_uint64(), C.c_uint64()
        a, b, s = C.c_void_p(), C.c_void_p(), C.c_void_p()
        _check(lib().kmx_result_part_view_device(self._h, part, C.byref(dev), C.byref(qb), C.byref(qe), C.byref(a), C.byref(b), C.byref(s)))
        return int(dev.value), int(qb.value), int(qe.value), a.value, b.value, s.value

    def counts(self):
        v = [C.c_uint64() for _ in range(6)]
        _check(lib().kmx_result_counts(self._h, *[C.byref(x) for x in v]))
        return dict(zip(["nq", "n_hits", "n_exact", "n_stitch", "n_prefix", "n_error"], [int(x.value) for x in v]))

    def paths(self):
        v = ResultPathInfo()
        v.struct_size = C.sizeof(ResultPathInfo)
        _check(lib().kmx_result_paths(self._h, C.byref(v)))
        return {"small": bool(v.small), "lookup_items": int(v.lookup_items), "lookup_pairs": bool(v.lookup_pairs),
                "deferred_long": bool(v.deferred_long), "tile_q_source": int(v.tile_q_source), "spec_fill": bool(v.spec_fill),
                "spec_ok": bool(v.spec_ok), "fill_blocks": int(v.fill_blocks), "fill_tiles": int(v.fill_tiles),
                "prefix_plain": int(v.prefix_plain), "prefix_small": int(v.prefix_small), "prefix_merge_small": int(v.prefix_merge_small),
                "prefix_mid": int(v.prefix_mid), "prefix_long": int(v.prefix_long), "prefix_large_chunks": int(v.prefix_large_chunks),
                "prefix_large_elems": int(v.prefix_large_elems)}

    def host(self, copy=True):
        c = self.counts()
        a, b, s, k = C.c_void_p(), C.c_void_p(), C.c_void_p(), C.c_void_p()
        _check(lib().kmx_result_view(self._h, C.byref(a), C.byref(b), C.byref(s), C.byref(k)))
        nq = c["nq"]
        hit_off = _view(a.value, nq + 1, np.uint64)
        n_pos = int(hit_off[nq]) if b.value else 0
        out = (hit_off, _view(b.value, n_pos, np.uint32), _view(s.value, nq, np.uint8), _view(k.value, nq, np.uint8))
        return tuple(x.copy() for x in out) if copy else out

    def device_ptrs(self):
        a, b, s = C.c_void_p(), C.c_void_p(), C.c_void_p()
        _check(lib().kmx_result_view_device(self._h, C.byref(a), C.byref(b), C.byref(s)))
        return a.value, b.value, s.value

    def device_tensors(self, device):
        import torch

        class _Arr:
            def __init__(self, ptr, n, typestr):
                self.__cuda_array_interface__ = {"shape": (int(n),), "typestr": typestr, "data": (int(ptr), False), "version": 2}

        c = self.counts()
        a, b, _ = self.device_ptrs()
        t_off = torch.as_tensor(_Arr(a, c["nq"] + 1, "<i8"), device=device)
        t_pos = torch.as_tensor(_Arr(b, c["n_hits"], "<i4"), device=device) if c["n_hits"] else torch.empty(0, dtype=torch.int32, device=device)
        return t_off, t_pos

    def gather_device(self, dst_device):
        a, b, s = C.c_void_p(), C.c_void_p(), C.c_void_p()
        _check(lib().kmx_result_gather_device(self._h, int(dst_device), C.byref(a), C.byref(b), C.byref(s)))
        return a.value, b.value, s.value

    def masks(self):
        c = self.counts()
        a, b, cc, d = C.c_void_p(), C.c_void_p(), C.c_void_p(), C.c_void_p()
        _check(lib().kmx_result_masks(self._h, C.byref(a), C.byref(b), C.byref(cc), C.byref(d)))
        nq = c["nq"]
        base = _view(a.value, nq, np.uint64).copy()
        cnt = _view(cc.value, nq, np.uint32).copy()
        src = _view(d.value, nq, np.uint64).copy()
        return base, b.value, cnt, src

    def close(self):
        if self._h:
            lib().kmx_result_free(self._h)
            self._h = C.c_void_p()
        self._index = None

    def __del__(self):
        try:
            self.close()
        except Exception:
            pass


class ApproxResult:

    def __init__(self):
        self._h = C.c_void_p()

    def counts(self):
        nq, hits, cand, chunks = C.c_uint64(), C.c_uint64(), C.c_uint64(), C.c_uint32()
        _check(lib().kmx_approx_counts(self._h, C.byref(nq), C.byref(hits), C.byref(cand), C.byref(chunks)))
        return {"nq": int(nq.value), "n_hits": int(hits.value), "n_candidates": int(cand.value), "n_chunks": int(chunks.value)}

    def host(self):
        c = self.counts()
        a, b, m, s = C.c_void_p(), C.c_void_p(), C.c_void_p(), C.c_void_p()
        _check(lib().kmx_approx_view(self._h, C.byref(a), C.byref(b), C.byref(m), C.byref(s)))
        nq, nh = c["nq"], c["n_hits"]
        out = (_view(a.value, nq + 1, np.uint64), _view(b.value, nh, np.uint32), _view(m.value, nh, np.uint8), _view(s.value, nq, np.uint8))
        return tuple(x.copy() for x in out)

    def lengths(self):
        p = C.c_void_p()
        _check(lib().kmx_approx_lengths(self._h, C.byref(p)))
        return _view(p.value, self.counts()["n_hits"], np.uint32).copy()

    def strands(self):
        p = C.c_void_p()
        _check(lib().kmx_approx_strands(self._h, C.byref(p)))
        return _view(p.value, self.counts()["n_hits"], np.uint8).copy()

    def found(self):
        p = C.c_void_p()
        _check(lib().kmx_approx_found(self._h, C.byref(p)))
        return _view(p.value, self.counts()["nq"], np.uint64).copy()

    def close(self):
        if self._h:
            lib().kmx_approx_free(self._h)
            self._h = C.c_void_p()

    def __del__(self):
        try:
            self.close()
        except Exception:
            pass


class Index:

    def __init__(self, ranks, sigma, ks, table=TABLE_AUTO, device=-1, n_threads=0, keep_host_arena=False,
                 query_size_range=0, host_flatten=False, aligned_copy=True, devices=None, prefix_levels=0):
        ranks = np.ascontiguousarray(ranks, np.uint8)
        ks = np.ascontiguousarray(ks, np.uint32)
        self.ks = ks.tolist()
        self.sigma = int(sigma)
        self.n = int(ranks.size)
        o = Options()
        o.struct_size = C.sizeof(Options)
        o.device = device
        o.table_kind = table
        o.n_threads = n_threads
        o.query_size_range = query_size_range
        o.keep_host_arena = int(keep_host_arena)
        o.host_flatten = int(host_flatten)
        o.no_aligned_copy = int(not aligned_copy)
        o.prefix_levels = int(prefix_levels)
        _set_devices(o, devices)
        self._h = C.c_void_p()
        _check(lib().kmx_index_build(ranks.ctypes.data, ranks.size, self.sigma, ks.ctypes.data, ks.size,
                                     C.byref(o), C.byref(self._h)))

    @classmethod
    def load(cls, path, device=-1, keep_host_arena=False, devices=None, prefix_levels=0):
        self = cls.__new__(cls)
        o = Options()
        o.struct_size = C.sizeof(Options)
        o.device = device
        o.keep_host_arena = int(keep_host_arena)
        o.prefix_levels = int(prefix_levels)
        _set_devices(o, devices)
        self._h = C.c_void_p()
        _check(lib().kmx_index_load(os.fsencode(path), C.byref(o), C.byref(self._h)))
        info = self.info()
        self.ks, self.sigma, self.n = info["ks"], info["sigma"], info["n"]
        return self

    def save(self, path):
        _check(lib().kmx_index_save(self._h, os.fsencode(path)))

    def info(self):
        n, sigma, nks, dbytes = C.c_uint64(), C.c_uint32(), C.c_uint32(), C.c_uint64()
        ks = np.zeros(KMX_MAX_KS, np.uint32)
        tk = np.zeros(KMX_MAX_KS, np.uint32)
        _check(lib().kmx_index_info(self._h, C.byref(n), C.byref(sigma), C.byref(nks), ks.ctypes.data, tk.ctypes.data, C.byref(dbytes)))
        return {"n": n.value, "sigma": sigma.value, "ks": ks[:nks.value].tolist(), "tables": tk[:nks.value].tolist(),
                "device_bytes": dbytes.value}

    def memory(self):
        v = [C.c_uint64() for _ in range(5)]
        _check(lib().kmx_index_memory(self._h, *[C.byref(x) for x in v]))
        return dict(zip(["positions", "aligned_copy", "cells", "prefix_levels", "tables"], [int(x.value) for x in v]))

    def paths(self):
        v = IndexPathInfo()
        v.struct_size = C.sizeof(IndexPathInfo)
        _check(lib().kmx_index_paths(self._h, C.byref(v)))
        return {"fill_slots": int(v.fill_slots), "fill_nontemporal": bool(v.fill_nontemporal), "rec64": bool(v.rec64),
                "tiny_cells": bool(v.tiny_cells), "scan_tile": int(v.scan_tile), "cell_shift": [int(v.cell_shift[i]) for i in range(v.n_ks)]}

    def devices(self):
        n = C.c_uint32()
        d = (C.c_int32 * KMX_MAX_DEVICES)()
        _check(lib().kmx_index_devices(self._h, C.byref(n), d))
        return [int(d[i]) for i in range(n.value)]

    def levels(self):
        lv = np.zeros(KMX_MAX_KS, np.uint32)
        _check(lib().kmx_index_levels(self._h, lv.ctypes.data))
        return lv[:len(self.ks)].tolist()

    def bucket_host(self, k, ranks):
        ranks = np.ascontiguousarray(ranks, np.uint8)
        if ranks.size != k:
            raise ValueError("bucket_host: k letters expected")
        p, n = C.c_void_p(), C.c_uint32()
        _check(lib().kmx_index_bucket_host(self._h, int(k), ranks.ctypes.data, C.byref(p), C.byref(n)))
        return _view(p.value, n.value, np.uint32).copy() if p.value else None

    def extend_query_size_range(self, new_maximum):
        _check(lib().kmx_index_extend_query_size_range(self._h, new_maximum))

    def arena_host(self):
        p, n = C.c_void_p(), C.c_uint64()
        _check(lib().kmx_index_arena_host(self._h, C.byref(p), C.byref(n)))
        return _view(p.value, n.value, np.uint32)

    def search(self, qranks, qoff, flags=SEARCH_DEFAULT, result=None):
        qranks = np.ascontiguousarray(qranks, np.uint8)
        qoff = np.ascontiguousarray(qoff, np.uint64)
        r = result or Result()
        _check(lib().kmx_search_batch(self._h, qranks.ctypes.data if qranks.size else None, qoff.ctypes.data,
                                      qoff.size - 1, flags, C.byref(r._h)))
        r._index = self
        return r

    def search_approx(self, qranks, qoff, max_subst, edit=False, strands=False, complement=None, loci=False, best=False, max_hits=0):
        qranks = np.ascontiguousarray(qranks, np.uint8)
        qoff = np.ascontiguousarray(qoff, np.uint64)
        r = ApproxResult()
        comp = None
        if strands:
            comp = np.ascontiguousarray(complement_table(self.sigma) if complement is None else complement, np.uint8)
            if comp.size != self.sigma:
                raise ValueError("search_approx: the complement table needs sigma entries")
        if loci or best or max_hits:
            flags = (APPROX_EDIT if edit else 0) | (APPROX_LOCI if loci else 0) | (APPROX_BEST if best else 0)
            o = ApproxOptions(C.sizeof(ApproxOptions), int(max_subst), flags, int(max_hits), comp.ctypes.data if strands else None)
            _check(lib().kmx_search_approx_opts(self._h, qranks.ctypes.data if qranks.size else None, qoff.ctypes.data, qoff.size - 1,
                                                C.byref(o), C.byref(r._h)))
            return r
        if strands:
            _check(lib().kmx_search_approx_strands(self._h, qranks.ctypes.data if qranks.size else None, qoff.ctypes.data,
                                                   qoff.size - 1, int(max_subst), APPROX_EDIT if edit else 0, comp.ctypes.data, C.byref(r._h)))
            return r
        _check(lib().kmx_search_approx(self._h, qranks.ctypes.data if qranks.size else None, qoff.ctypes.data,
                                       qoff.size - 1, int(max_subst), APPROX_EDIT if edit else 0, C.byref(r._h)))
        return r

    def text(self):
        n = int(self.info()["n"])
        out = np.zeros(n, np.uint8)
        _check(lib().kmx_index_text(self._h, out.ctypes.data, n, None))
        return out

    def text_packed_bytes(self):
        b = C.c_uint64()
        _check(lib().kmx_index_text(self._h, None, 0, C.byref(b)))
        return int(b.value)

    def search_device(self, d_qranks_ptr, d_qoff_ptr, nq, flags=SEARCH_DEFAULT, stream=0, result=None):
        r = result or Result()
        _check(lib().kmx_search_batch_device(self._h, d_qranks_ptr, d_qoff_ptr, nq, flags, stream or None, C.byref(r._h)))
        r._index = self
        return r

    def debug_words(self):
        w = np.zeros(16, np.uint64)
        _check(lib().kmx_debug_words(self._h, w.ctypes.data))
        return w

    def stats_enable(self, on=True):
# ... 26 lines not shown
```

Measured before the change: 7064.

## Add compact per-sector byte-count table for k-mer lookup probes

Builds a compact lookup structure at index build time when it is small enough (at most about 2 MB) and almost no bucket count reaches 255. It stores one byte-sized count per key plus one 32-bit base per 64-key sector. The lookup kernel reads the 64-byte sector and the sector base, then rebuilds the arena offset with SWAR prefix sums and a SAD instruction. It falls back to the full offset table when a saturated count appears in the prefix. The aim is to replace reads of the larger 32-bit offset table with a table about a quarter of the size that stays in cache better. The cost is wider per-query loads, extra ALU work, and a lower occupancy bound on the compact kernel variant.

Measured after the change: 6762. 0.957x the previous value.

```diff
diff --git a/include/kmx.h b/include/kmx.h
--- a/include/kmx.h
+++ b/include/kmx.h
@@ -140,6 +140,8 @@
     uint32_t scan_tile;
     uint32_t n_ks;
     uint32_t cell_shift[KMX_MAX_KS];
+    uint32_t lookup_compact[KMX_MAX_KS];
+    uint64_t lookup_compact_bytes;
 } kmx_index_path_info;
 kmx_status kmx_index_paths(const kmx_index* index, kmx_index_path_info* out);
 
@@ -161,6 +163,9 @@
     uint32_t prefix_long;
     uint32_t prefix_large_chunks;
     uint64_t prefix_large_elems;
+    uint64_t lookup_fallbacks;
+    uint32_t lookup_compact;
+    uint32_t reserved0;
 } kmx_result_path_info;
 #define KMX_TILE_Q_NONE 0u
 #define KMX_TILE_Q_PARTITION 1u
diff --git a/kmer_index_amd/csrc/kmx_capi.hip b/kmer_index_amd/csrc/kmx_capi.hip
--- a/kmer_index_amd/csrc/kmx_capi.hip
+++ b/kmer_index_amd/csrc/kmx_capi.hip
@@ -180,6 +180,7 @@
     KmxIndexDev h_header{};
     kmx::FillVariant fill_variant{12, true};
     bool rec32 = true;
+    uint64_t bytes_lcompact = 0;
     bool tiny_cells = false;
     bool broken = false;
     std::vector<uint32_t> host_arena;
@@ -231,7 +232,7 @@
     bool last_had_long = false;
     bool last_had_pairs = false;
     struct PathRec { uint32_t small = 0, items = 0, pairs = 0, defer_long = 0, tile_q_source = 0, spec_fill = 0, spec_ok = 0, fill_blocks = 0, fill_tiles = 0;
-                     uint32_t p_plain = 0, p_small = 0, p_merge = 0, p_mid = 0, p_long = 0, p_chunks = 0; uint64_t p_elems = 0; };
+                     uint32_t p_plain = 0, p_small = 0, p_merge = 0, p_mid = 0, p_long = 0, p_chunks = 0; uint64_t p_elems = 0; uint64_t lookup_fallbacks = 0; uint32_t compact = 0; };
     PathRec path;
     std::shared_ptr<ResultPool> pool;
     SearchCtx ctx;
@@ -493,6 +494,36 @@
             if ((st = upload(ix, im.slots.data(), im.slots.size(), &el.slots)) != KMX_OK) return bail(st);
             if ((st = upload(ix, im.ukeys.data(), im.ukeys.size(), &el.ukeys)) != KMX_OK) return bail(st);
         }
+        el.lcnt8 = nullptr; el.lbase = nullptr;
+        if (el.atab) {
+            const uint64_t n_sectors = (im.n_keys + 63) / 64;
+            const uint64_t bytes = n_sectors * 64 + (n_sectors + 1) * 4;
+            int force = -1;
+            if (const char* e = getenv("KMX_LOOKUP_COMPACT")) { if (e[0] == '0' && !e[1]) force = 0; else if (e[0] == '1' && !e[1]) force = 1; }
+            if (force == 1 || (force < 0 && bytes <= (uint64_t(2) << 20))) {
+                void *pc = nullptr, *pb = nullptr, *pn = nullptr;
+                unsigned int n_big = 0;
+                hipError_t ce = hipMalloc(&pc, n_sectors * 64 + 64);
+                if (ce == hipSuccess) ce = hipMalloc(&pb, (n_sectors + 1) * 4 + 64);
+                if (ce == hipSuccess) ce = hipMalloc(&pn, 64);
+                if (ce == hipSuccess) ce = hipMemset(pn, 0, 64);
+                if (ce == hipSuccess) {
+                    kmx::launch_build_lcompact(nullptr, el.atab, im.n_keys, static_cast<uint8_t*>(pc), static_cast<uint32_t*>(pb), static_cast<unsigned int*>(pn));
+                    ce = hipGetLastError();
+                }
+                if (ce == hipSuccess) ce = hipMemcpy(&n_big, pn, sizeof n_big, hipMemcpyDeviceToHost);
+                if (pn) (void)hipFree(pn);
+                if (ce == hipSuccess && (force == 1 || uint64_t(n_big) * 100 < im.n_keys)) {
+                    ix->allocs.push_back(pc); ix->allocs.push_back(pb);
+                    ix->device_bytes += bytes; ix->bytes_lcompact += bytes;
+                    el.lcnt8 = static_cast<const uint8_t*>(pc); el.lbase = static_cast<const uint32_t*>(pb);
+                } else {
+                    if (pc) (void)hipFree(pc);
+                    if (pb) (void)hipFree(pb);
+                    if (ce != hipSuccess) { fail(ce == hipErrorOutOfMemory ? KMX_ERR_OUT_OF_MEMORY : KMX_ERR_HIP, std::string("compact probe table: ") + hipGetErrorString(ce)); return bail(KMX_ERR_HIP); }
+                }
+            }
+        }
         el.dir = nullptr; el.dir_shift = 0; el.n_dir = 0;
         if (im.table_kind == KMX_TABLE_OPEN && el.n_ukeys >= 1024) {
             uint32_t key_bits = 1;
@@ -573,6 +604,7 @@
     ix->ks = src->ks; ix->table_kinds = src->table_kinds; ix->elem_sizes = src->elem_sizes; ix->tail = src->tail;
     ix->fill_variant = src->fill_variant; ix->rec32 = src->rec32; ix->tiny_cells = src->tiny_cells;
     ix->bytes_positions = src->bytes_positions; ix->bytes_aligned = src->bytes_aligned; ix->bytes_cells = src->bytes_cells; ix->bytes_levels = src->bytes_levels;
+    ix->bytes_lcompact = src->bytes_lcompact;
     auto bail = [&](kmx_status s) { std::string keep = g_err; kmx_index_free(ix); g_err = keep; return s; };
     hipError_t e = hipSetDevice(device);
     if (e != hipSuccess) { fail(KMX_ERR_NO_DEVICE, std::string("replica device: ") + hipGetErrorString(e)); return bail(KMX_ERR_NO_DEVICE); }
@@ -623,6 +655,11 @@
         de.dir = static_cast<const uint32_t*>(p);
         if (!clone(se.cnt8, se.cnt8 ? size_t(se.n_keys) : 0, 64, &p)) return bail(st);
         de.cnt8 = static_cast<const uint8_t*>(p);
+        const size_t n_sectors = size_t((se.n_keys + 63) / 64);
+        if (!clone(se.lcnt8, se.lcnt8 ? n_sectors * 64 : 0, 64, &p)) return bail(st);
+        de.lcnt8 = static_cast<const uint8_t*>(p);
+        if (!clone(se.lbase, se.lbase ? (n_sectors + 1) * 4 : 0, 64, &p)) return bail(st);
+        de.lbase = static_cast<const uint32_t*>(p);
     }
     if (!clone(nullptr, 0, 0, &p)) return bail(st);
     {
@@ -1294,6 +1331,8 @@
     v.scan_tile = uint32_t(kmx::scan_tile());
     v.n_ks = uint32_t(ix->ks.size());
     for (size_t i = 0; i < ix->ks.size(); ++i) v.cell_shift[i] = ix->h_header.elems[i].cnt8 ? ix->h_header.elems[i].cell_shift : 0u;
+    for (size_t i = 0; i < ix->ks.size(); ++i) v.lookup_compact[i] = ix->h_header.elems[i].lcnt8 ? 1u : 0u;
+    v.lookup_compact_bytes = ix->bytes_lcompact;
     v.struct_size = std::min<uint32_t>(out->struct_size, uint32_t(sizeof v));
     memcpy(out, &v, v.struct_size);
     return KMX_OK;
@@ -1310,6 +1349,7 @@
     v.fill_blocks = r->path.fill_blocks; v.fill_tiles = r->path.fill_tiles;
     v.prefix_plain = r->path.p_plain; v.prefix_small = r->path.p_small; v.prefix_merge_small = r->path.p_merge; v.prefix_mid = r->path.p_mid;
     v.prefix_long = r->path.p_long; v.prefix_large_chunks = r->path.p_chunks; v.prefix_large_elems = r->path.p_elems;
+    v.lookup_fallbacks = r->path.lookup_fallbacks; v.lookup_compact = r->path.compact;
     v.struct_size = std::min<uint32_t>(out->struct_size, uint32_t(sizeof v));
     memcpy(out, &v, v.struct_size);
     return KMX_OK;
@@ -1444,9 +1484,10 @@
     const int items = force_items ? (force_items == 8 ? 8 : 4) : (!pairs && ix->tiny_cells) ? 8 : 4;
     const bool defer_long = r->last_had_long;
     const uint32_t lflags = (flags & ~KMX_SEARCH_INTERNAL_DEFER_LONG) | (defer_long ? KMX_SEARCH_INTERNAL_DEFER_LONG : 0u);
-    r->path.items = uint32_t(items); r->path.pairs = pairs; r->path.defer_long = defer_long;
+    const bool compact = !pairs && ix->bytes_lcompact != 0;
+    r->path.items = uint32_t(items); r->path.pairs = pairs; r->path.defer_long = defer_long; r->path.compact = compact;
     timed(ix, K_LOOKUP, s, [&] {
-        kmx::launch_lookup(s, items, pairs, dix, qr, qo, nq, d, ctr, r->bsum.as<uint64_t>(), lflags);
+        kmx::launch_lookup(s, items, pairs, compact, dix, qr, qo, nq, d, ctr, r->bsum.as<uint64_t>(), lflags);
         if (defer_long) kmx::launch_lookup_long(s, dix, qr, qo, nq, d, ctr, flags);
     });
     const kmx::FillVariant fv = kmx::effective_fill_variant(ix->fill_variant, ix->rec32);
@@ -1529,6 +1570,7 @@
     const uint64_t max_runs = r->h_ctr[KMX_CTR_MAX_RUNS];
     {
         const uint64_t n_merge = r->h_ctr[KMX_CTR_PREFIX_MERGE], n_mid = r->h_ctr[KMX_CTR_PREFIX_MID];
+        r->path.lookup_fallbacks = r->h_ctr[KMX_CTR_LOOKUP_FALLBACK];
         r->path.p_plain = uint32_t(r->h_ctr[KMX_CTR_PREFIX_PLAIN]);
         r->path.p_merge = uint32_t(n_merge);
         r->path.p_small = uint32_t(n_prefix_small - std::min(n_prefix_small, n_merge));
diff --git a/kmer_index_amd/csrc/kmx_kernels.h b/kmer_index_amd/csrc/kmx_kernels.h
--- a/kmer_index_amd/csrc/kmx_kernels.h
+++ b/kmer_index_amd/csrc/kmx_kernels.h
@@ -22,7 +22,7 @@
 };
 
 uint64_t lookup_blocks(uint64_t nq, int items);
-void launch_lookup(hipStream_t s, int items, bool pairs, const KmxIndexDev* ix, const uint8_t* qranks, const uint64_t* qoff,
+void launch_lookup(hipStream_t s, int items, bool pairs, bool compact, const KmxIndexDev* ix, const uint8_t* qranks, const uint64_t* qoff,
                    uint64_t nq, const QueryDesc& d, unsigned long long* ctr, uint64_t* block_hits, uint32_t flags);
 void launch_lookup_long(hipStream_t s, const KmxIndexDev* ix, const uint8_t* qranks, const uint64_t* qoff, uint64_t nq, const QueryDesc& d,
                         unsigned long long* ctr, uint32_t flags);
@@ -35,6 +35,7 @@
 void launch_build_dir(hipStream_t s, const uint64_t* d_ukeys, uint64_t n_ukeys, uint32_t shift, uint32_t n_dir, uint32_t* d_dir);
 void launch_build_cells(hipStream_t s, const uint32_t* d_offs, const uint32_t* d_region, uint64_t n_keys, uint32_t cell_shift,
                         uint32_t* d_cells, uint8_t* d_cnt8);
+void launch_build_lcompact(hipStream_t s, const uint32_t* d_atab, uint64_t n_keys, uint8_t* d_lcnt8, uint32_t* d_lbase, unsigned int* d_n_big);
 
 struct SparseTables {
     uint64_t* d_ukeys = nullptr;
diff --git a/kmer_index_amd/csrc/kmx_kernels.hip b/kmer_index_amd/csrc/kmx_kernels.hip
--- a/kmer_index_amd/csrc/kmx_kernels.hip
+++ b/kmer_index_amd/csrc/kmx_kernels.hip
@@ -429,7 +429,7 @@
 
 struct BlockCounters {
     unsigned int n_long, base_long;
-    unsigned int n_stitch, n_stitch_tiny, n_stitch_short, n_resolved, n_prefix, n_prefix_big, n_prefix_merge, n_prefix_mid, n_prefix_plain, n_error, n_none, n_more;
+    unsigned int n_stitch, n_stitch_tiny, n_stitch_short, n_resolved, n_prefix, n_prefix_big, n_prefix_merge, n_prefix_mid, n_prefix_plain, n_error, n_none, n_more, n_fallback;
     unsigned long long words, pelems, hits;
     unsigned int max_runs;
     unsigned int base_stitch, base_stitch_tiny, base_stitch_short, base_prefix, base_prefix_big;
@@ -513,13 +513,42 @@
     return r;
 }
 
+__device__ __forceinline__ const char* compact_first_addr(const KmxElemDev* el, uint64_t h)
+{
+    return reinterpret_cast<const char*>(el->lcnt8 + (h & ~uint64_t(63)));
+}
+__device__ __forceinline__ bool compact_finish(const KmxElemDev* el, uint64_t h, const u32x4_a1 (&sec)[4], uint32_t base, Run& r)
+{
+    const uint32_t p = uint32_t(h) & 63u;
+    const uint32_t full = (p + 1u) >> 2;
+    const uint32_t part = (1u << (((p + 1u) & 3u) * 8u)) - 1u;
+    uint32_t lines4 = 0, ff = 0, cw = 0;
+#pragma unroll
+    for (uint32_t i = 0; i < 16; ++i) {
+        const uint32_t w = sec[i >> 2][i & 3];
+        const uint32_t t = w & (i < full ? 0xFFFFFFFFu : i == full ? part : 0u);
+        ff |= (~t - 0x01010101u) & t;
+        lines4 += ((t >> 5) & 0x07070707u) + ((((t & 0x1F1F1F1Fu) + 0x1F1F1F1Fu) >> 5) & 0x01010101u);
+        cw = i == (p >> 2) ? w : cw;
+    }
+    if (ff & 0x80808080u) return false;
+    const uint32_t c = (cw >> ((p & 3u) * 8u)) & 0xFFu;
+    const uint32_t before = __builtin_amdgcn_sad_u8(lines4, 0u, 0u) - ((c + 31u) >> 5);
+    r.src = el->arena_base + (uint64_t(base + before) << 5);
+    r.cnt = c;
+    return true;
+}
+
 #define KMX_PLAN_LDS 256
 
 #ifndef KMX_LOOKUP_OCC
 #define KMX_LOOKUP_OCC 4
 #endif
-template <int ITEMS, bool PAIRS>
-__global__ __launch_bounds__(KMX_BLOCK, PAIRS ? KMX_LOOKUP_OCC : (ITEMS > 4 ? 4 : 5)) void k_lookup(const KmxIndexDev* __restrict__ ix,
+#ifndef KMX_LOOKUP_COMPACT_OCC
+#define KMX_LOOKUP_COMPACT_OCC 4
+#endif
+template <int ITEMS, bool PAIRS, bool COMPACT>
+__global__ __launch_bounds__(KMX_BLOCK, PAIRS ? KMX_LOOKUP_OCC : (ITEMS > 4 ? 4 : (COMPACT ? KMX_LOOKUP_COMPACT_OCC : 5))) void k_lookup(const KmxIndexDev* __restrict__ ix,
                                                       const uint8_t* __restrict__ qranks,
                                                       const uint64_t* __restrict__ qoff, uint64_t nq,
                                                       QueryDesc d, unsigned long long* __restrict__ ctr,
@@ -531,7 +560,7 @@
     static_assert(KMX_PLAN_LDS == KMX_BLOCK, "one planner entry per thread");
     if (threadIdx.x == 0) {
         bc.n_long = 0;
-        bc.n_stitch = bc.n_stitch_tiny = bc.n_stitch_short = bc.n_resolved = bc.n_prefix = bc.n_prefix_big = bc.n_prefix_merge = bc.n_prefix_mid = bc.n_prefix_plain = bc.n_error = bc.n_none = bc.n_more = 0;
+        bc.n_stitch = bc.n_stitch_tiny = bc.n_stitch_short = bc.n_resolved = bc.n_prefix = bc.n_prefix_big = bc.n_prefix_merge = bc.n_prefix_mid = bc.n_prefix_plain = bc.n_error = bc.n_none = bc.n_more = bc.n_fallback = 0;
         bc.words = bc.pelems = bc.hits = 0;
         bc.max_runs = 0;
         unsigned int j = 0;
@@ -677,6 +706,12 @@
         uint64_t ha[ITEMS], hb[ITEMS];
         bool oka[ITEMS], okb[ITEMS];
         u32x4_a1 pa[ITEMS], pb[ITEMS];
+        static_assert(!(COMPACT && PAIRS), "the compact probe is the lean variants'");
+        constexpr bool CP_EARLY = COMPACT && ITEMS == 4, CP_LATE = COMPACT && ITEMS != 4;
+        bool cpa[ITEMS];
+        u32x4_a1 pc[CP_EARLY ? ITEMS : 1][3];
+        uint32_t pl[CP_EARLY ? ITEMS : 1];
+        unsigned int n_fallback = 0;
 #pragma unroll
         for (int it = 0; it < ITEMS; ++it) {
             const KmxElemDev* ela = &elems_s[eab[it] & 0xFF];
@@ -689,7 +724,17 @@
                 oka[it] = hash16<false>(wa[it], done[it] ? ela->k : 0u, sigma, ha[it]);
                 if (PAIRS) okb[it] = hash16<false>(wb[it], two[it] ? elb->k : 0u, sigma, hb[it]);
             }
-            pa[it] = *(const KMX_GLOBAL u32x4_a1*)((done[it] && oka[it]) ? probe_first_addr(ela, ha[it]) : reinterpret_cast<const char*>(dummy));
+            cpa[it] = COMPACT && done[it] && oka[it] && ela->lcnt8 != nullptr;
+            pa[it] = *(const KMX_GLOBAL u32x4_a1*)((done[it] && oka[it] && !(CP_LATE && cpa[it]))
+                                                       ? (CP_EARLY && cpa[it] ? compact_first_addr(ela, ha[it]) : probe_first_addr(ela, ha[it]))
+                                                       : reinterpret_cast<const char*>(dummy));
+            if (CP_EARLY) {
+                const int ci = CP_EARLY ? it : 0;
+                const char* rest = cpa[it] ? compact_first_addr(ela, ha[it]) + 16 : reinterpret_cast<const char*>(dummy);
+#pragma unroll
+                for (int j = 0; j < 3; ++j) pc[ci][j] = *(const KMX_GLOBAL u32x4_a1*)(rest + 16 * j);
+                pl[ci] = *(const KMX_GLOBAL uint32_t*)(cpa[it] ? reinterpret_cast<const char*>(ela->lbase + (ha[it] >> 6)) : reinterpret_cast<const char*>(dummy));
+            }
             if (PAIRS) pb[it] = *(const KMX_GLOBAL u32x4_a1*)((two[it] && okb[it]) ? probe_first_addr(elb, hb[it]) : reinterpret_cast<const char*>(dummy));
         }
         struct Pend {
@@ -707,7 +752,31 @@
             Run ra{0, 0}, rb{0, 0};
             if (done[it]) {
                 const KmxElemDev* ela = &elems_s[eab[it] & 0xFF];
-                if (oka[it]) ra = probe_finish(ela, ha[it], pa[it]);
+                if (oka[it]) {
+                    if (COMPACT && cpa[it]) {
+                        u32x4_a1 sec[4];
+                        uint32_t line0;
+                        if (CP_EARLY) {
+                            const int ci = CP_EARLY ? it : 0;
+                            sec[0] = pa[it]; sec[1] = pc[ci][0]; sec[2] = pc[ci][1]; sec[3] = pc[ci][2];
+                            line0 = pl[ci];
+                        } else {
+                            const char* sp = compact_first_addr(ela, ha[it]);
+#pragma unroll
+                            for (int j = 0; j < 4; ++j) sec[j] = *(const KMX_GLOBAL u32x4_a1*)(sp + 16 * j);
+                            line0 = as_global(ela->lbase)[ha[it] >> 6];
+                        }
+                        if (!compact_finish(ela, ha[it], sec, line0, ra)) {
+                            const KMX_GLOBAL uint32_t* atab = as_global(ela->atab);
+                            const uint32_t e0 = atab[ha[it]], e1 = atab[ha[it] + 1];
+                            ra.src = ela->arena_base + (e0 & ~31u);
+                            ra.cnt = atab_count(e0, e1);
+                            ++n_fallback;
+                        }
+                    } else {
+                        ra = probe_finish(ela, ha[it], pa[it]);
+                    }
+                }
                 if (!PAIRS || !two[it]) {
                     const uint8_t status = oka[it] ? KMX_Q_OK : KMX_Q_BAD_RANK;
                     n_err += status != KMX_Q_OK;
@@ -801,6 +870,7 @@
         }
         if (n_err) atomicAdd(&bc.n_error, n_err);
         if (n_none) atomicAdd(&bc.n_none, n_none);
+        if (n_fallback) atomicAdd(&bc.n_fallback, n_fallback);
     }
 
 #pragma unroll 1
@@ -857,6 +927,7 @@
         if (bc.n_resolved) atomicAdd(&ctr[KMX_CTR_STITCH_RESOLVED], (unsigned long long)bc.n_resolved);
         if (bc.n_error) atomicAdd(&ctr[KMX_CTR_ERROR], (unsigned long long)bc.n_error);
         if (bc.n_none) atomicAdd(&ctr[KMX_CTR_NONE], (unsigned long long)bc.n_none);
+        if (bc.n_fallback) atomicAdd(&ctr[KMX_CTR_LOOKUP_FALLBACK], (unsigned long long)bc.n_fallback);
     }
     __syncthreads();
 #pragma unroll
@@ -3219,13 +3290,15 @@
 
 uint64_t lookup_blocks(uint64_t nq, int items) { return blocks_for(nq, uint64_t(KMX_BLOCK) * uint64_t(items)); }
 
-void launch_lookup(hipStream_t s, int items, bool pairs, const KmxIndexDev* ix, const uint8_t* qranks, const uint64_t* qoff,
+void launch_lookup(hipStream_t s, int items, bool pairs, bool compact, const KmxIndexDev* ix, const uint8_t* qranks, const uint64_t* qoff,
                    uint64_t nq, const QueryDesc& d, unsigned long long* ctr, uint64_t* block_hits, uint32_t flags)
 {
     const dim3 grid(blocks_for(nq, uint64_t(KMX_BLOCK) * uint64_t(items))), block(KMX_BLOCK);
-    if (pairs) hipLaunchKernelGGL((k_lookup<4, true>), grid, block, 0, s, ix, qranks, qoff, nq, d, ctr, block_hits, flags);
-    else if (items == 8) hipLaunchKernelGGL((k_lookup<8, false>), grid, block, 0, s, ix, qranks, qoff, nq, d, ctr, block_hits, flags);
-    else hipLaunchKernelGGL((k_lookup<4, false>), grid, block, 0, s, ix, qranks, qoff, nq, d, ctr, block_hits, flags);
+    if (pairs) hipLaunchKernelGGL((k_lookup<4, true, false>), grid, block, 0, s, ix, qranks, qoff, nq, d, ctr, block_hits, flags);
+    else if (items == 8 && compact) hipLaunchKernelGGL((k_lookup<8, false, true>), grid, block, 0, s, ix, qranks, qoff, nq, d, ctr, block_hits, flags);
+    else if (items == 8) hipLaunchKernelGGL((k_lookup<8, false, false>), grid, block, 0, s, ix, qranks, qoff, nq, d, ctr, block_hits, flags);
+    else if (compact) hipLaunchKernelGGL((k_lookup<4, false, true>), grid, block, 0, s, ix, qranks, qoff, nq, d, ctr, block_hits, flags);
+    else hipLaunchKernelGGL((k_lookup<4, false, false>), grid, block, 0, s, ix, qranks, qoff, nq, d, ctr, block_hits, flags);
 }
 
 void launch_validate(hipStream_t s, const KmxIndexDev* ix, const uint32_t* arena, const uint8_t* qranks, const uint64_t* qoff,
@@ -4507,6 +4580,25 @@
     else if (h == n_keys) atab[h] = end & ~31u;
 }
 
+__global__ __launch_bounds__(KMX_BLOCK) void k_build_lcompact(const uint32_t* __restrict__ atab, uint64_t n_keys, uint8_t* __restrict__ lcnt8,
+                                                              uint32_t* __restrict__ lbase, unsigned int* __restrict__ n_big)
+{
+    const uint64_t h = uint64_t(blockIdx.x) * KMX_BLOCK + threadIdx.x;
+    const uint64_t n_padded = (n_keys + 63) & ~uint64_t(63);
+    uint32_t c = 0;
+    if (h < n_keys) c = atab_count(atab[h], atab[h + 1]);
+    if (h < n_padded) lcnt8[h] = uint8_t(min(c, 255u));
+    if (h <= n_padded && (h & 63) == 0) lbase[h >> 6] = atab[min(h, n_keys)] >> 5;
+    const uint64_t big = __ballot(c >= 255u);
+    if (lane_id() == 0 && big) atomicAdd(n_big, (unsigned int)__popcll(big));
+}
+
+void launch_build_lcompact(hipStream_t s, const uint32_t* d_atab, uint64_t n_keys, uint8_t* d_lcnt8, uint32_t* d_lbase, unsigned int* d_n_big)
+{
+    hipLaunchKernelGGL(k_build_lcompact, dim3(blocks_for(((n_keys + 63) & ~uint64_t(63)) + 1, KMX_BLOCK)), dim3(KMX_BLOCK), 0, s, d_atab, n_keys,
+                       d_lcnt8, d_lbase, d_n_big);
+}
+
 __global__ __launch_bounds__(KMX_BLOCK) void k_build_aligned_copy(const uint32_t* __restrict__ offs,
                                                                   const uint32_t* __restrict__ aoffs, uint64_t n_keys,
                                                                   uint32_t* __restrict__ region)
diff --git a/kmer_index_amd/csrc/kmx_types.h b/kmer_index_amd/csrc/kmx_types.h
--- a/kmer_index_amd/csrc/kmx_types.h
+++ b/kmer_index_amd/csrc/kmx_types.h
@@ -33,6 +33,8 @@
     uint32_t n_levels;
     uint64_t lvl_offs_at[KMX_MAX_LEVELS];
     uint64_t lvl_base[KMX_MAX_LEVELS];
+    const uint8_t* lcnt8;
+    const uint32_t* lbase;
 };
 
 enum { KMX_SCHEME_NONE = 0, KMX_SCHEME_SINGLE = 1, KMX_SCHEME_MULTI = 2, KMX_SCHEME_REPLANNED = 3 };
@@ -147,6 +149,7 @@
     KMX_CTR_PSB_BANDS = 20,
     KMX_CTR_PSB_CUTS = 21,
     KMX_CTR_PSB_SPLITS = 22,
+    KMX_CTR_LOOKUP_FALLBACK = 26,
     KMX_CTR_COUNT = 28
 };
 #define KMX_LONG_PARTS 256
diff --git a/kmer_index_amd/engine.py b/kmer_index_amd/engine.py
--- a/kmer_index_amd/engine.py
+++ b/kmer_index_amd/engine.py
@@ -55,7 +55,8 @@
 
 class IndexPathInfo(C.Structure):
     _fields_ = [("struct_size", C.c_uint32), ("fill_slots", C.c_uint32), ("fill_nontemporal", C.c_uint32), ("rec64", C.c_uint32),
-                ("tiny_cells", C.c_uint32), ("scan_tile", C.c_uint32), ("n_ks", C.c_uint32), ("cell_shift", C.c_uint32 * KMX_MAX_KS)]
+                ("tiny_cells", C.c_uint32), ("scan_tile", C.c_uint32), ("n_ks", C.c_uint32), ("cell_shift", C.c_uint32 * KMX_MAX_KS),
+                ("lookup_compact", C.c_uint32 * KMX_MAX_KS), ("lookup_compact_bytes", C.c_uint64)]
 
 
 class ResultPathInfo(C.Structure):
@@ -63,7 +64,8 @@
                 ("deferred_long", C.c_uint32), ("tile_q_source", C.c_uint32), ("spec_fill", C.c_uint32), ("spec_ok", C.c_uint32),
                 ("fill_blocks", C.c_uint32), ("fill_tiles", C.c_uint32),
                 ("prefix_plain", C.c_uint32), ("prefix_small", C.c_uint32), ("prefix_merge_small", C.c_uint32), ("prefix_mid", C.c_uint32),
-                ("prefix_long", C.c_uint32), ("prefix_large_chunks", C.c_uint32), ("prefix_large_elems", C.c_uint64)]
+                ("prefix_long", C.c_uint32), ("prefix_large_chunks", C.c_uint32), ("prefix_large_elems", C.c_uint64),
+                ("lookup_fallbacks", C.c_uint64), ("lookup_compact", C.c_uint32), ("reserved0", C.c_uint32)]
 
 
 _lib = None
@@ -264,7 +266,8 @@
                 "spec_ok": bool(v.spec_ok), "fill_blocks": int(v.fill_blocks), "fill_tiles": int(v.fill_tiles),
                 "prefix_plain": int(v.prefix_plain), "prefix_small": int(v.prefix_small), "prefix_merge_small": int(v.prefix_merge_small),
                 "prefix_mid": int(v.prefix_mid), "prefix_long": int(v.prefix_long), "prefix_large_chunks": int(v.prefix_large_chunks),
-                "prefix_large_elems": int(v.prefix_large_elems)}
+                "prefix_large_elems": int(v.prefix_large_elems), "lookup_fallbacks": int(v.lookup_fallbacks),
+                "lookup_compact": bool(v.lookup_compact)}
 
     def host(self, copy=True):
         c = self.counts()
@@ -427,7 +430,8 @@
         v.struct_size = C.sizeof(IndexPathInfo)
         _check(lib().kmx_index_paths(self._h, C.byref(v)))
         return {"fill_slots": int(v.fill_slots), "fill_nontemporal": bool(v.fill_nontemporal), "rec64": bool(v.rec64),
-                "tiny_cells": bool(v.tiny_cells), "scan_tile": int(v.scan_tile), "cell_shift": [int(v.cell_shift[i]) for i in range(v.n_ks)]}
+                "tiny_cells": bool(v.tiny_cells), "scan_tile": int(v.scan_tile), "cell_shift": [int(v.cell_shift[i]) for i in range(v.n_ks)],
+                "lookup_compact": [bool(v.lookup_compact[i]) for i in range(v.n_ks)], "lookup_compact_bytes": int(v.lookup_compact_bytes)}
 
     def devices(self):
         n = C.c_uint32()
```
